# juanmc2005/diart

Hardware: NVIDIA H100
Metric: audio-seconds/sec (real-time factor) at 5s/0.5s step, batch 256 (higher is better)
Workload: dtype f32

## Files before the change

diart_b200/_lib.py:

```python
from __future__ import annotations

import ctypes as C
import os
from typing import Dict, Optional

import numpy as np
import torch

_HERE = os.path.dirname(os.path.abspath(__file__))
LIB_PATH = os.path.join(_HERE, "libdiartb200.so")

_lib: Optional[C.CDLL] = None


class DgTensor(C.Structure):
    _fields_ = [("name", C.c_char_p), ("data", C.c_void_p), ("numel", C.c_int64)]


_P = C.c_void_p
SIGNATURES = {
    "dg_last_error": (C.c_char_p, []),
    "dg_version": (C.c_int, []),
    "dg_launch_count": (C.c_int64, []),
    "dg_profile_enable": (C.c_int, [C.c_int]),
    "dg_profile_report": (C.c_int, [C.c_char_p, C.c_int]),
    "dg_selftest_gemm_tc": (C.c_int, [C.c_int, C.c_int, C.c_int, C.c_int, C.c_int, C.c_int, C.POINTER(C.c_float),
                                      C.POINTER(C.c_float)]),
    "dg_selftest_gemm_tc_grid": (C.c_int, [C.c_int, C.c_int, C.c_int, C.c_int, C.c_int, C.c_int, C.POINTER(C.c_int)]),
    "dg_selftest_gemm_tc_bounds": (C.c_int, [C.c_int, C.c_int, C.c_int, C.c_int, C.POINTER(C.c_int), C.POINTER(C.c_int),
                                             C.POINTER(C.c_int)]),
    "dg_selftest_wgmma_row_shift": (C.c_int, [C.c_int, C.POINTER(C.c_uint)]),
    "dg_selftest_gemm_tc_halo": (C.c_int, [C.c_int, C.c_int, C.c_int, C.c_int, C.c_int, C.c_int, C.POINTER(C.c_int),
                                           C.POINTER(C.c_int)]),
    "dg_selftest_split_f16_host": (C.c_int, [_P, C.c_longlong, _P, _P]),
    "dg_seg_create": (C.c_int, [C.POINTER(DgTensor), C.c_int, C.c_int, C.POINTER(_P)]),
    "dg_seg_dims": (C.c_int, [_P, C.c_int, C.POINTER(C.c_int), C.POINTER(C.c_int)]),
    "dg_seg_set_powerset": (C.c_int, [_P, C.c_int, C.c_int]),
    "dg_seg_forward": (C.c_int, [_P, _P, C.c_int, C.c_int, _P, _P]),
    "dg_seg_destroy": (C.c_int, [_P]),
    "dg_emb_create": (C.c_int, [C.POINTER(DgTensor), C.c_int, C.c_int, C.c_int, C.POINTER(_P)]),
    "dg_emb_dims": (C.c_int, [_P, C.c_int, C.POINTER(C.c_int), C.POINTER(C.c_int)]),
    "dg_emb_forward": (C.c_int, [_P, _P, _P, C.c_int, C.c_int, C.c_int, C.c_int, C.c_int, C.c_float, _P, _P]),
    "dg_emb_forward_rows": (C.c_int, [_P, _P, _P, C.c_int, C.c_int, C.c_int, _P, _P]),
    "dg_emb_destroy": (C.c_int, [_P]),
    "dg_emb_debug_trunk": (C.c_int, [_P, _P, C.c_int, C.c_int, C.c_int, _P, C.c_int64, _P]),
    "dg_seg_debug_stage": (C.c_int, [_P, _P, C.c_int, C.c_int, C.c_int, C.c_int, _P, C.c_int64, _P]),
    "dg_emb_debug_stage": (C.c_int, [_P, _P, _P, C.c_int, C.c_int, C.c_int, C.c_int, C.c_int, C.c_int, _P, C.c_int64, _P]),
    "dg_selftest_sinc_filters_host": (C.c_int, [_P, _P, _P]),
    "dg_selftest_fbank_tables_host": (C.c_int, [_P, _P]),
    "dg_osp": (C.c_int, [_P, C.c_int, C.c_int, C.c_int, C.c_float, C.c_float, C.c_int, _P, _P]),
    "dg_normalize_embeddings": (C.c_int, [_P, C.c_int, C.c_int, C.c_float, _P, _P]),
    "dg_cluster_create": (C.c_int, [C.c_int, C.c_int, C.c_double, C.c_double, C.c_double, C.c_int, C.POINTER(_P)]),
    "dg_cluster_set_metric": (C.c_int, [_P, C.c_int]),
    "dg_cluster_step": (C.c_int, [_P, _P, _P, C.c_int, C.c_int, C.c_int, _P, _P, _P]),
    "dg_cluster_reset": (C.c_int, [_P]),
    "dg_cluster_get_state": (C.c_int, [_P, _P, _P, C.POINTER(C.c_int)]),
    "dg_cluster_set_state": (C.c_int, [_P, _P, _P, C.c_int]),
    "dg_cluster_destroy": (C.c_int, [_P]),
    "dg_cluster_record_len": (C.c_int, [_P]),
    "dg_cluster_export_delta": (C.c_int, [_P, _P, _P]),
    "dg_cluster_merge": (C.c_int, [_P, _P, C.c_int, C.c_int, _P, C.c_int, _P]),
    "dg_pipeline_identity_export": (C.c_int, [_P, _P, _P]),
    "dg_pipeline_identity_merge": (C.c_int, [_P, _P, C.c_int, C.c_int, _P]),
    "dg_pipeline_create": (C.c_int, [_P, _P, _P, C.c_float, C.c_float, C.c_int, C.POINTER(_P)]),
    "dg_pipeline_set_hop": (C.c_int, [_P, C.c_int]),
    "dg_pipeline_step": (C.c_int, [_P, _P, C.c_int, C.c_int, _P, _P, _P, _P, _P]),
    "dg_pipeline_step_host": (C.c_int, [_P, _P, C.c_int, C.c_int, _P, _P, _P, _P]),
    "dg_pipeline_submit": (C.c_int, [_P, _P, C.c_int, C.c_int, _P]),
    "dg_pipeline_collect": (C.c_int, [_P, C.POINTER(_P), C.POINTER(_P), C.POINTER(_P), _P]),
    "dg_pipeline_collect_copy": (C.c_int, [_P, _P, _P, _P, _P]),
    "dg_pipeline_submit_host": (C.c_int, [_P, _P, C.c_int, C.c_int]),
    "dg_pipeline_collect_host": (C.c_int, [_P, _P, _P, _P]),
    "dg_pipeline_destroy": (C.c_int, [_P]),
    "dg_pipeline_nets_sets": (C.c_int, [_P, _P, C.c_int, C.c_int, C.c_int, _P, _P, _P, _P, C.c_int64, _P]),
    "dg_post_create": (C.c_int, [C.c_int, C.c_int, C.c_int, C.c_int, _P, C.c_double, C.c_int, C.POINTER(_P)]),
    "dg_post_step": (C.c_int, [_P, _P, _P, C.c_int, _P, _P, _P, C.c_int, C.POINTER(C.c_int), _P]),
    "dg_post_reset": (C.c_int, [_P]),
    "dg_post_destroy": (C.c_int, [_P]),
    "dg_stream_create": (C.c_int, [C.c_int, C.c_int, C.c_int, C.c_int, C.POINTER(_P)]),
    "dg_stream_push_host": (C.c_int, [_P, _P, C.c_int]),
    "dg_stream_available": (C.c_int, [_P]),
    "dg_stream_windows": (C.c_int, [_P, C.c_int, _P, _P]),
    "dg_stream_reset": (C.c_int, [_P]),
    "dg_stream_destroy": (C.c_int, [_P]),
    "dg_pipeline_submit_stream": (C.c_int, [_P, _P, C.c_int]),
    "dg_pipeline_call_stream": (C.c_int, [_P, _P, _P, C.c_int, _P, _P, _P, C.c_int, C.POINTER(C.c_int), _P, _P]),
    "dg_pipeline_call_host": (C.c_int, [_P, _P, _P, C.c_int, C.c_int, _P, _P, _P, C.c_int, C.POINTER(C.c_int), _P, _P]),
    "dg_pipeline_last_call_h2d_bytes": (C.c_int64, [_P]),
    "dg_resample_create": (C.c_int, [C.c_int, C.c_int, _P, C.c_int, C.c_int, C.POINTER(_P)]),
    "dg_resample_out_len": (C.c_int64, [_P, C.c_int64]),
    "dg_resample_forward": (C.c_int, [_P, _P, C.c_int, C.c_int64, _P, _P]),
    "dg_resample_destroy": (C.c_int, [_P]),
    "dg_stream_create_resampled": (C.c_int, [C.c_int, C.c_int, _P, C.c_int, C.c_int, C.POINTER(_P)]),
    "dg_stream_crop_host": (C.c_int, [_P, C.c_int, _P, _P]),
    "dg_sweep_create": (C.c_int, [C.c_int, C.c_int, C.c_int, C.c_int, C.c_int, _P, C.c_int, C.POINTER(_P)]),
    "dg_sweep_run": (C.c_int, [_P, _P, _P, C.c_int, _P, C.c_int, _P, _P, _P, _P, _P, C.c_int, C.POINTER(C.c_int), _P]),
    "dg_sweep_destroy": (C.c_int, [_P]),
    "dg_sweep_set_scored_regions": (C.c_int, [_P, C.c_int, _P, _P]),
    "dg_sweep_set_trial_sets": (C.c_int, [_P, C.c_int, _P, C.c_int]),
    "dg_sweep_set_seeds": (C.c_int, [_P, C.c_int, _P, _P]),
    "dg_sweep_set_identities": (C.c_int, [_P, C.c_int, _P]),
    "dg_sweep_score": (C.c_int, [_P, _P, _P, C.c_int, _P, C.c_int, _P, _P, _P, C.c_double, C.c_double, _P, _P, C.c_int,
                                 C.c_int, _P, _P, _P, C.c_int, _P]),
    "dg_sweep_run_files": (C.c_int, [_P, _P, _P, C.c_int, C.c_int, _P, _P, C.c_int, _P, _P, _P, _P, _P, C.c_int,
                                     C.POINTER(C.c_int), _P]),
    "dg_sweep_score_files": (C.c_int, [_P, _P, _P, C.c_int, C.c_int, _P, _P, C.c_int, _P, _P, _P, _P, C.c_double, _P, _P,
                                       _P, _P, _P, _P, _P, C.c_int, _P]),
    "dg_sweep_state_order": (C.c_int, [C.c_int, _P, C.c_int, _P]),
    "dg_sweep_run_latencies": (C.c_int, [_P, _P, _P, C.c_int, C.c_int, _P, C.c_int, C.c_int, _P, _P, _P, C.c_int, _P, _P,
                                         _P, _P, C.c_int, C.POINTER(C.c_int), _P]),
    "dg_sweep_score_latencies": (C.c_int, [_P, _P, _P, C.c_int, C.c_int, _P, C.c_int, C.c_int, _P, _P, _P, C.c_int, _P, _P,
                                           _P, _P, C.c_double, _P, _P, _P, _P, _P, _P]),
    "dg_sweep_check_latencies": (C.c_int, [C.c_int, C.c_int, _P, C.c_int, C.c_int, _P, _P, _P, C.c_int, C.c_int]),
    "dg_vad_sweep_curve_latencies": (C.c_int, [_P, _P, C.c_int, C.c_int, _P, C.c_int, C.c_int, _P, _P, _P, _P]),
    "dg_vad_sweep_create": (C.c_int, [C.c_int, C.c_int, C.c_int, _P, C.c_int, C.POINTER(_P)]),
    "dg_vad_sweep_curve": (C.c_int, [_P, _P, C.c_int, C.c_int, _P, _P, _P]),
    "dg_vad_sweep_run_files": (C.c_int, [_P, _P, C.c_int, _P, _P, C.c_int, C.POINTER(C.c_int), _P]),
    "dg_vad_sweep_score_files": (C.c_int, [_P, _P, C.c_int, _P, _P, _P, C.c_double, _P, _P, _P, _P]),
    "dg_vad_sweep_destroy": (C.c_int, [_P]),
    "dg_vad_sweep_set_scored_regions": (C.c_int, [_P, C.c_int, _P, _P]),
    "dg_multi_create": (C.c_int, [_P, _P, C.c_int, C.c_int, C.c_int, C.c_int, C.c_int, C.c_double, C.c_double, C.c_double,
                                  C.c_float, C.c_float, C.c_int, C.c_int, _P, C.POINTER(_P)]),
    "dg_multi_create_vad": (C.c_int, [_P, C.c_int, C.c_int, C.c_int, C.c_int, C.c_double, C.c_int, _P, C.POINTER(_P)]),
    "dg_multi_open": (C.c_int, [_P, C.c_int]),
    "dg_multi_close": (C.c_int, [_P, C.c_int]),
    "dg_multi_push_host": (C.c_int, [_P, C.c_int, _P, C.c_int]),
    "dg_multi_available": (C.c_int, [_P, C.c_int]),
    "dg_multi_step": (C.c_int, [_P, _P, C.c_int, _P, _P, _P, C.c_int, C.POINTER(C.c_int), _P, _P, _P]),
    "dg_multi_last_step_ms": (C.c_int, [_P, C.POINTER(C.c_float)]),
    "dg_multi_destroy": (C.c_int, [_P]),
    "dg_selftest_multi_staging_host": (C.c_int, [C.c_int, C.c_int, C.c_int, _P, _P, _P, _P]),
    "dg_multi_add_rate": (C.c_int, [_P, _P, C.c_int, C.c_int, C.POINTER(C.c_int)]),
    "dg_multi_open_rate": (C.c_int, [_P, C.c_int, C.c_int]),
    "dg_multi_open_config": (C.c_int, [_P, C.c_int, C.c_int, C.c_int, _P]),
    "dg_multi_open_seeded": (C.c_int, [_P, C.c_int, C.c_int, C.c_int, _P, _P, C.c_int]),
    "dg_multi_get_state": (C.c_int, [_P, C.c_int, _P, _P, C.POINTER(C.c_int)]),
    "dg_multi_last_windows": (C.c_int, [_P, _P, C.c_int]),
    "dg_gallery_create": (C.c_int, [_P, C.c_int, C.c_int, C.c_int, C.POINTER(_P)]),
    "dg_gallery_destroy": (C.c_int, [_P]),
    "dg_gallery_query": (C.c_int, [_P, _P, C.c_int, _P, _P, C.c_double, _P, _P, _P]),
    "dg_multi_set_gallery": (C.c_int, [_P, _P, C.c_double]),
    "dg_multi_set_names": (C.c_int, [_P, C.c_int, C.c_uint32, _P]),
    "dg_multi_set_slot_gallery": (C.c_int, [_P, C.c_int, _P, C.c_double]),
    "dg_selftest_gallery_plan_host": (C.c_int, [C.c_int, _P, C.c_int, _P, _P, _P, _P, _P, C.c_int, _P]),
    "dg_selftest_multi_gallery_host": (C.c_int, [C.c_int, C.c_int, C.c_int, C.c_int, _P, C.c_int, _P, _P, C.c_char_p,
                                                 C.c_int]),
    "dg_multi_last_names": (C.c_int, [_P, _P, C.c_int, C.POINTER(C.c_int)]),
    "dg_selftest_multi_frames_host": (C.c_int, [C.c_int, C.c_int, C.c_int, C.c_int, C.c_int, _P, C.c_int, _P, _P, _P, C.c_int,
                                                C.POINTER(C.c_int)]),
    "dg_multi_export_bytes": (C.c_int, [_P, _P, C.c_int, _P]),
    "dg_multi_export": (C.c_int, [_P, _P, C.c_int, C.c_int, _P, C.c_int64]),
    "dg_multi_import": (C.c_int, [_P, _P, C.c_int64, C.c_int, _P, _P]),
    "dg_selftest_multi_transfer_host": (C.c_int, [_P, C.c_int, _P, _P, _P, C.c_int, C.c_int, _P, _P, _P, C.c_int64, _P,
                                                  C.c_char_p, C.c_int]),
}


class DiartB200Error(RuntimeError):
    pass


def lib() -> C.CDLL:
    global _lib
    if _lib is not None:
        return _lib
    from . import build as _build

    if not os.path.exists(LIB_PATH) or (_build._stale() and _build.have_nvcc()):
        _build.build()
    try:
        handle = C.CDLL(LIB_PATH)
    except OSError as e:
        raise DiartB200Error(f"cannot load {LIB_PATH}: {e}. Run `python -m diart_b200.build`.") from e
    for name, (res, args) in SIGNATURES.items():
        fn = getattr(handle, name)
        fn.restype, fn.argtypes = res, args
    _lib = handle
    return handle


def check(rc: int):
    if rc == 0:
        return
    msg = lib().dg_last_error().decode()
    if rc == -1:
        if "Cannot update unknown centers" in msg:
            raise AssertionError(msg)
        raise ValueError(msg)
    if rc == -3:
        raise KeyError(msg)
    raise DiartB200Error(f"libdiartb200 error {rc}: {msg}")


def require_cuda(device: torch.device):
    if device.type != "cuda":
        raise DiartB200Error(
            f"diart_b200 runs on CUDA devices only (got '{device}'); there is no CPU implementation")
    if not torch.cuda.is_available():
        raise DiartB200Error("diart_b200 needs a CUDA device (sm_90a); none is available")


def pack_state_dict(state: Dict[str, "torch.Tensor | np.ndarray"]):
    keep, items = [], []
    for name, value in state.items():
        arr = value.detach().cpu().numpy() if isinstance(value, torch.Tensor) else np.asarray(value)
        if arr.dtype.kind != "f":
            continue
        arr = np.ascontiguousarray(arr, dtype=np.float32)
        bname = name.encode()
        keep.extend([arr, bname])
        items.append(DgTensor(bname, arr.ctypes.data, arr.size))
    array = (DgTensor * len(items))(*items)
    keep.append(array)
    return array, len(items), keep


def stream_ptr(device: torch.device) -> int:
    return torch.cuda.current_stream(device).cuda_stream


def ptr(t: Optional[torch.Tensor]) -> Optional[int]:
    return None if t is None else t.data_ptr()
```

diart_b200/csrc/api.cu:

```cuda
#include <math.h>
#include <stdlib.h>
#include <string.h>

#include <map>
#include <sstream>
#include <vector>

#include "host.cuh"

namespace dg {

static thread_local std::string g_err;
std::atomic<long long> g_launches{0};
thread_local int g_sm_limit = 0;
void set_error(const std::string& msg) { g_err = msg; }

struct ProfRec {
  std::string name;
  cudaEvent_t a, b;
};
static bool g_prof = false;
static std::vector<ProfRec> g_recs;
static const bool g_trace = getenv("DG_TRACE_LAUNCHES") && getenv("DG_TRACE_LAUNCHES")[0] == '1';
ProfScope::ProfScope(const char* name_, cudaStream_t st_) : on(g_prof), st(st_), a(nullptr), b(nullptr), name(name_) {
  if (g_trace) first = g_launches.load();
  if (!on) return;
  cudaEventCreate(&a);
  cudaEventCreate(&b);
  cudaEventRecord(a, st);
}
ProfScope::~ProfScope() {
  if (g_trace) fprintf(stderr, "dg-trace %s %lld %lld\n", name, first, (long long)g_launches.load());
  if (!on) return;
  cudaEventRecord(b, st);
  g_recs.push_back({name, a, b});
}

int upload_u16(DevBuf& b, const std::vector<uint16_t>& h) {
  if (b.ensure(h.size() * 2)) return -2;
  DG_CUDA(cudaMemcpy(b.p, h.data(), h.size() * 2, cudaMemcpyHostToDevice));
  return 0;
}

int upload_split(WeightPlanes& w, const std::vector<float>& w_nk, int N, int Npad, int K) {
  std::vector<uint16_t> h((size_t)Npad * K), l((size_t)Npad * K);
  w.scale = weight_plane_scale(w_nk.data(), (size_t)N * K);
  w.Npad = Npad;
  w.K = K;
  split_weights_host(w_nk.data(), N, Npad, K, h.data(), l.data(), w.scale);
  return (upload_u16(w.hi, h) || upload_u16(w.lo, l)) ? DG_ECUDA : 0;
}

int set_weights(TcGemm& t, const WeightPlanes& w) {
  if (t.KW * t.Cin != w.K) {
    set_error(std::string(t.tag ? t.tag : "gemm_tc") + ": the launch reads K = " + std::to_string(t.KW * t.Cin) +
              " but the weight planes have K = " + std::to_string(w.K));
    return DG_EINVAL;
  }
  t.W_hi = w.hi.p;
  t.W_lo = w.lo.p;
  t.w_scale = w.scale;
  t.Npad = w.Npad;
  return 0;
}

int upload(DevBuf& b, const std::vector<float>& h) {
  if (b.ensure(h.size() * sizeof(float))) return -2;
  DG_CUDA(cudaMemcpy(b.p, h.data(), h.size() * sizeof(float), cudaMemcpyHostToDevice));
  return 0;
}

}

extern "C" const char* dg_last_error(void) { return g_err.c_str(); }
extern "C" int dg_version(void) { return 100; }
extern "C" int64_t dg_launch_count(void) { return (int64_t)g_launches.load(); }

extern "C" int dg_profile_enable(int enable) {
  g_prof = enable != 0;
  return DG_OK;
}

extern "C" int dg_profile_report(char* buf, int cap) {
  cudaDeviceSynchronize();
  std::map<std::string, std::pair<int, double>> agg;
  for (auto& r : g_recs) {
    float ms = 0.f;
    cudaEventElapsedTime(&ms, r.a, r.b);
    auto& e = agg[r.name];
    e.first++;
    e.second += ms;
    cudaEventDestroy(r.a);
    cudaEventDestroy(r.b);
  }
  g_recs.clear();
  std::ostringstream os;
  os << "{";
  bool first = true;
  for (auto& kv : agg) {
    if (!first) os << ", ";
    first = false;
    os << "\"" << kv.first << "\": {\"count\": " << kv.second.first << ", \"ms\": " << kv.second.second << "}";
  }
  os << "}";
  const std::string s = os.str();
  if (!buf || cap <= (int)s.size()) {
    set_error("dg_profile_report: buffer too small");
    return DG_EINVAL;
  }
  memcpy(buf, s.c_str(), s.size() + 1);
  return (int)s.size();
}

extern "C" int dg_selftest_split_f16_host(const float* x, long long n, unsigned short* hi, unsigned short* lo) {
  if (!x || !hi || !lo || n < 0) {
    set_error("dg_selftest_split_f16_host: null argument");
    return DG_EINVAL;
  }
  for (long long i = 0; i < n; i++) {
    hi[i] = host_f32_to_h16(x[i]);
    lo[i] = host_f32_to_h16(x[i] - host_h16_to_f32(hi[i]));
  }
  return DG_OK;
}

extern "C" int dg_selftest_gemm_tc(int M, int Cin, int KW, int dil, int N, int epi, float* max_abs_diff,
                                   float* out_rms) {
  if (M < 1 || Cin < 16 || Cin % 16 || KW < 1 || N % 4 || !max_abs_diff || !out_rms) {
    set_error("dg_selftest_gemm_tc: bad arguments");
    return DG_EINVAL;
  }
  const int K = KW * Cin, npad = N == 64 ? 64 : (N + 255) / 256 * 256;
  const long long Mtot = M;
  std::vector<float> A((size_t)Mtot * Cin), Wkn((size_t)K * N), Wnk((size_t)N * K), bias(N), bsc(N), bsh(N);
  uint32_t seed = 12345u;
  auto rnd = [&]() {
    seed = seed * 1664525u + 1013904223u;
    return ((seed >> 8) & 0xFFFF) / 65536.f - 0.5f;
  };
  static const float amp = getenv("DG_SELFTEST_AMP") ? (float)atof(getenv("DG_SELFTEST_AMP")) : 2.f;
  for (auto& v : A) v = amp * rnd();
  for (int k = 0; k < K; k++)
    for (int n = 0; n < N; n++) {
      const float w = rnd() * 0.25f;
      Wkn[(size_t)k * N + n] = w;
      Wnk[(size_t)n * K + k] = w;
    }
  for (int n = 0; n < N; n++) {
    bias[n] = rnd();
    bsc[n] = 1.f + rnd();
    bsh[n] = rnd();
  }
  DevBuf dA, dWkn, dB, dS, dH, dAh, dAl, dC0, dC1, dOh, dOl;
  WeightPlanes dW;
  if (upload(dA, A) || upload(dWkn, Wkn) || upload(dB, bias) || upload(dS, bsc) || upload(dH, bsh) ||
      upload_split(dW, Wnk, N, npad, K))
    return DG_ECUDA;
  if (dAh.ensure((size_t)Mtot * Cin * 2) || dAl.ensure((size_t)Mtot * Cin * 2) || dC0.ensure((size_t)M * N * 4) ||
      dC1.ensure((size_t)M * N * 4) || dOh.ensure((size_t)M * N * 2) || dOl.ensure((size_t)M * N * 2))
    return DG_ECUDA;
  int rc;
  GemmArgs g{};
  g.A = dA.as<float>(); g.lda = Cin; g.Cin = Cin; g.KW = KW; g.dil = dil; g.Mtot = Mtot; g.M = M;
  g.W = dWkn.as<float>(); g.ldw = N; g.N = N; g.bias = dB.as<float>(); g.bn_scale = dS.as<float>();
  g.bn_shift = dH.as<float>(); g.C = dC0.as<float>(); g.ldc = N; g.epi = epi == 0 ? EPI_BIAS : EPI_BIAS_LEAKY_BN;
  g.tag = "selftest_simt";
  if ((rc = launch_gemm(g, nullptr))) return rc;
  if ((rc = launch_split_ex(dA.as<float>(), Mtot, Cin, Cin, Cin, 0, 1, nullptr, nullptr, dAh.p, dAl.p, nullptr))) return rc;
  TcGemm t{};
  t.A_hi = dAh.p; t.A_lo = dAl.p; t.lda = Cin; t.Cin = Cin; t.KW = KW; t.dil = dil; t.Mtot = Mtot; t.M = M;
  t.N = N; t.bias = dB.as<float>(); t.bn_scale = dS.as<float>();
  t.bn_shift = dH.as<float>(); t.out_f32 = dC1.as<float>(); t.out_hi = dOh.p; t.out_lo = dOl.p; t.ldc = N;
  t.epi = epi; t.tag = "selftest_tc";
  if ((rc = set_weights(t, dW)) || (rc = launch_gemm_tc(t, nullptr))) return rc;
  DG_CUDA(cudaDeviceSynchronize());
  std::vector<float> c0((size_t)M * N), c1((size_t)M * N);
  DG_CUDA(cudaMemcpy(c0.data(), dC0.p, c0.size() * 4, cudaMemcpyDeviceToHost));
  std::vector<uint16_t> oh, ol;
  if (epi == 1) {
    oh.resize((size_t)M * N);
    ol.resize((size_t)M * N);
    DG_CUDA(cudaMemcpy(oh.data(), dOh.p, oh.size() * 2, cudaMemcpyDeviceToHost));
    DG_CUDA(cudaMemcpy(ol.data(), dOl.p, ol.size() * 2, cudaMemcpyDeviceToHost));
    for (size_t i = 0; i < c1.size(); i++) c1[i] = host_h16_to_f32(oh[i]) + host_h16_to_f32(ol[i]);
  } else {
    DG_CUDA(cudaMemcpy(c1.data(), dC1.p, c1.size() * 4, cudaMemcpyDeviceToHost));
  }
  double md = 0, ss = 0;
  size_t worst = 0, n_big = 0;
  for (size_t i = 0; i < c0.size(); i++) {
    const double d = fabs((double)c0[i] - (double)c1[i]);
    if (!(d <= md)) {
      md = d;
      worst = i;
    }
    if (!(d <= 1e-2)) n_big++;
    ss += (double)c0[i] * c0[i];
  }
  if (n_big)
    fprintf(stderr, "dg_selftest_gemm_tc: %zu of %zu outputs differ by more than 1e-2; worst at row %zu col %zu: simt %g, wgmma %g\n",
            n_big, c0.size(), worst / N, worst % N, c0[worst], c1[worst]);
  if (n_big && epi == 1) {
    size_t shown = 0;
    for (size_t i = 0; i < c0.size() && shown < 12; i++)
      if (!(fabs((double)c0[i] - (double)c1[i]) <= 1e-2)) {
        fprintf(stderr, "   row %zu col %zu: simt %g, planes hi 0x%04x lo 0x%04x\n", i / N, i % N, c0[i], oh[i], ol[i]);
        shown++;
      }
  }
  *max_abs_diff = (float)md;
  *out_rms = (float)sqrt(ss / c0.size());
  return DG_OK;
}

extern "C" int dg_selftest_gemm_tc_grid(int M, int Cin, int KW, int dil, int N, int epi, int* equal) {
  if (M < 1 || Cin % 64 || KW < 1 || KW > 9 || N < 1 || N % 4 || epi < 0 || epi > 5 || !equal ||
      (epi == 3 && (KW != 9 || dil < 3 || M % (dil * dil) || N % 32)) || (epi == 5 && (N > 64 || M % 888))) {
    set_error("dg_selftest_gemm_tc_grid: bad arguments");
    return DG_EINVAL;
  }
  const int K = KW * Cin;
  const int npad = epi == 5 || N == 64 ? 64 : (epi == 3 && N == 32 ? 32 : (N + 127) / 128 * 128);
  const int ldc = epi == 3 ? (N + 31) / 32 * 32 : N;
  const int item_rows = epi == 4 ? 296 : 888, tile_rows = epi == 5 ? gemm_tc_pool3_tile_rows(item_rows) : 128;
  const long long m_tiles = (M + tile_rows - 1) / tile_rows;
  uint32_t seed = 777u;
  auto rnd = [&]() {
    seed = seed * 1664525u + 1013904223u;
    return ((seed >> 8) & 0xFFFF) / 65536.f - 0.5f;
  };
  std::vector<float> A((size_t)M * Cin), Wnk((size_t)N * K), bias(N), bsc(N), bsh(N), res((size_t)M * ldc), pw((size_t)M * 4);
  for (auto& v : A) v = 2.f * rnd();
  for (auto& v : Wnk) v = 0.25f * rnd();
  for (int n = 0; n < N; n++) {
    bias[n] = rnd();
    bsc[n] = 1.f + rnd();
    bsh[n] = rnd();
  }
  for (auto& v : res) v = rnd();
  for (auto& v : pw) v = rnd() + 0.5f;
  const size_t f32_bytes = epi == 0 || epi == 2 ? (size_t)M * ldc * 4 : (epi == 5 ? (size_t)(M / 3) * ldc * 4 : 0);
  const size_t plane_bytes = epi == 1 || epi == 3 ? (size_t)M * ldc * 2 : 0;
  const size_t part_bytes = epi == 4 ? (size_t)m_tiles * 2 * TC_POOL_SLOTS * N * 4 : (epi == 5 ? (size_t)m_tiles * 2 * TC_POOL3_SLOTS * N * 4 : 0);
  DevBuf dA, dAh, dAl, dB, dS, dH, dRes, dRh, dRl, dPw, dF, dOh, dOl, dPart;
  WeightPlanes dW;
  if (upload(dA, A) || upload(dB, bias) || upload(dS, bsc) || upload(dH, bsh) || upload(dRes, res) || upload(dPw, pw) ||
      upload_split(dW, Wnk, N, npad, K))
    return DG_ECUDA;
  if (dAh.ensure((size_t)M * Cin * 2) || dAl.ensure((size_t)M * Cin * 2) || dRh.ensure((size_t)M * ldc * 2) ||
      dRl.ensure((size_t)M * ldc * 2) || dF.ensure(f32_bytes + 4) || dOh.ensure(plane_bytes + 4) ||
      dOl.ensure(plane_bytes + 4) || dPart.ensure(part_bytes + 4))
    return DG_ECUDA;
  int rc;
  if ((rc = launch_split_ex(dA.as<float>(), M, Cin, Cin, Cin, 0, 1, nullptr, nullptr, dAh.p, dAl.p, nullptr)) ||
      (rc = launch_split_ex(dRes.as<float>(), M, ldc, ldc, ldc, 0, 1, nullptr, nullptr, dRh.p, dRl.p, nullptr)))
    return rc;
  int taps[9];
  for (int j = 0; j < 9; j++) taps[j] = (j / 3 - 1) * dil + (j % 3 - 1);
  TcGemm t{};
  t.A_hi = dAh.p; t.A_lo = dAl.p; t.lda = Cin; t.Cin = Cin; t.KW = KW; t.dil = dil; t.Mtot = M; t.M = M;
  t.N = N; t.bias = dB.as<float>(); t.bn_scale = dS.as<float>(); t.bn_shift = dH.as<float>(); t.ldc = ldc;
  t.epi = epi; t.tag = "selftest_tc_grid";
  t.out_f32 = f32_bytes ? dF.as<float>() : nullptr;
  t.out_hi = plane_bytes ? dOh.p : nullptr;
  t.out_lo = plane_bytes ? dOl.p : nullptr;
  if (epi == 3) {
    t.tap_off = taps; t.Wp = t.Wop = t.Hp = t.Hop = dil; t.relu = 1;
    t.res_hi = dRh.p; t.res_lo = dRl.p;
  }
  if (epi == 4) {
    t.pool_w = dPw.as<float>(); t.pool_part = dPart.as<float>(); t.pool_item_rows = item_rows; t.pool_K = 3; t.pool_T = item_rows;
  }
  if (epi == 5) {
    t.pool_part = dPart.as<float>(); t.pool_item_rows = item_rows; t.pool3_T = item_rows / 3 - 2;
    t.pool3_tile_rows = tile_rows;
  }
  if ((rc = set_weights(t, dW))) return rc;
  std::vector<unsigned char> first, cur;
  *equal = 1;
  const int caps[4] = {0, 1, 3, 7};
  for (int ci = 0; ci < 4; ci++) {
    DG_CUDA(cudaMemset(dF.p, 0, f32_bytes + 4));
    DG_CUDA(cudaMemset(dOh.p, 0, plane_bytes + 4));
    DG_CUDA(cudaMemset(dOl.p, 0, plane_bytes + 4));
    DG_CUDA(cudaMemset(dPart.p, 0, part_bytes + 4));
    {
      SmLimit cap(caps[ci]);
      if ((rc = launch_gemm_tc(t, nullptr))) return rc;
    }
    DG_CUDA(cudaDeviceSynchronize());
    cur.resize(f32_bytes + 2 * plane_bytes + part_bytes);
    DG_CUDA(cudaMemcpy(cur.data(), dF.p, f32_bytes, cudaMemcpyDeviceToHost));
    DG_CUDA(cudaMemcpy(cur.data() + f32_bytes, dOh.p, plane_bytes, cudaMemcpyDeviceToHost));
    DG_CUDA(cudaMemcpy(cur.data() + f32_bytes + plane_bytes, dOl.p, plane_bytes, cudaMemcpyDeviceToHost));
    DG_CUDA(cudaMemcpy(cur.data() + f32_bytes + 2 * plane_bytes, dPart.p, part_bytes, cudaMemcpyDeviceToHost));
    if (ci == 0)
      first.swap(cur);
    else if (cur != first)
      *equal = 0;
  }
  return DG_OK;
}

extern "C" int dg_selftest_wgmma_row_shift(int base_offset_mode, unsigned* ok_shifts) {
  if (base_offset_mode < 0 || base_offset_mode > 1 || !ok_shifts) {
    set_error("dg_selftest_wgmma_row_shift: bad arguments");
    return DG_EINVAL;
  }
  return selftest_wgmma_row_shift(base_offset_mode, ok_shifts) ? DG_ECUDA : DG_OK;
}

extern "C" int dg_selftest_gemm_tc_halo(int M, int Cin, int KW, int dil, int N, int epi, int* equal, int* halo) {
  const bool folded = Cin % 64 != 0;
  if (M < 1 || Cin < 16 || Cin % 16 || Cin > 128 || KW < 2 || KW > 9 || dil < 1 || N < 1 || N % 4 ||
      (epi != 0 && epi != 1 && epi != 2 && epi != 5) || (epi == 1 && N % 32) || (epi == 5 && (N > 64 || M % 888)) ||
      (folded && dil != 1) || !equal || !halo) {
    set_error("dg_selftest_gemm_tc_halo: bad arguments");
    return DG_EINVAL;
  }
  const int K = KW * Cin, Kf = folded ? (K + 63) / 64 * 64 : K;
  const int npad = epi == 5 || N == 64 ? 64 : (N + 127) / 128 * 128;
  const int item_rows = 888, tile_rows = epi == 5 ? gemm_tc_pool3_tile_rows(item_rows) : 128;
  const long long m_tiles = (M + tile_rows - 1) / tile_rows;
  const long long tail = 64;
  uint32_t seed = 9090u;
  auto rnd = [&]() {
    seed = seed * 1664525u + 1013904223u;
    return ((seed >> 8) & 0xFFFF) / 65536.f - 0.5f;
  };
  std::vector<float> A((size_t)(M + tail) * Cin, 0.f), Wnk((size_t)N * K), Wf((size_t)N * Kf, 0.f), bias(N), bsc(N), bsh(N);
  for (size_t i = 0; i < (size_t)M * Cin; i++) A[i] = 2.f * rnd();
  for (auto& v : Wnk) v = 0.25f * rnd();
  for (int n = 0; n < N; n++)
    for (int k = 0; k < K; k++) Wf[(size_t)n * Kf + k] = Wnk[(size_t)n * K + k];
  for (int n = 0; n < N; n++) {
    bias[n] = rnd();
    bsc[n] = 1.f + rnd();
    bsh[n] = rnd();
  }
  const size_t f32_bytes = epi == 0 || epi == 2 ? (size_t)M * N * 4 : (epi == 5 ? (size_t)(M / 3) * N * 4 : 0);
  const size_t plane_bytes = epi == 1 ? (size_t)M * N * 2 : 0;
  const size_t part_bytes = epi == 5 ? (size_t)m_tiles * 2 * TC_POOL3_SLOTS * N * 4 : 0;
  DevBuf dA, dAh, dAl, dB, dS, dH, dF, dOh, dOl, dPart;
  WeightPlanes dW, dWf;
  if (upload(dA, A) || upload(dB, bias) || upload(dS, bsc) || upload(dH, bsh) || upload_split(dW, Wnk, N, npad, K) ||
      upload_split(dWf, Wf, N, npad, Kf))
    return DG_ECUDA;
  if (dAh.ensure((size_t)(M + tail) * Cin * 2) || dAl.ensure((size_t)(M + tail) * Cin * 2) || dF.ensure(f32_bytes + 4) ||
      dOh.ensure(plane_bytes + 4) || dOl.ensure(plane_bytes + 4) || dPart.ensure(part_bytes + 4))
    return DG_ECUDA;
  int rc;
  if ((rc = launch_split_ex(dA.as<float>(), M + tail, Cin, Cin, Cin, 0, 1, nullptr, nullptr, dAh.p, dAl.p, nullptr))) return rc;
  TcGemm t{};
  t.A_hi = dAh.p; t.A_lo = dAl.p; t.lda = Cin; t.Cin = Cin; t.KW = KW; t.dil = dil; t.Mtot = M; t.M = M;
  t.N = N; t.bias = dB.as<float>(); t.bn_scale = dS.as<float>(); t.bn_shift = dH.as<float>(); t.ldc = N;
  t.epi = epi; t.tag = "selftest_tc_halo";
  t.out_f32 = f32_bytes ? dF.as<float>() : nullptr;
  t.out_hi = plane_bytes ? dOh.p : nullptr;
  t.out_lo = plane_bytes ? dOl.p : nullptr;
  if (epi == 5) {
    t.pool_part = dPart.as<float>(); t.pool_item_rows = item_rows; t.pool3_T = item_rows / 3 - 2;
    t.pool3_tile_rows = tile_rows;
  }
  if ((rc = set_weights(t, dW))) return rc;
  *halo = gemm_tc_halo(t) ? 1 : 0;
  TcGemm ref = t;
  ref.tap_boxes = 1;
  if (folded) {
    ref.Cin = Kf;
    ref.KW = 1;
    if ((rc = set_weights(ref, dWf))) return rc;
  }
  std::vector<unsigned char> first, cur;
  *equal = 1;
  for (int run = 0; run < 3; run++) {
    DG_CUDA(cudaMemset(dF.p, 0, f32_bytes + 4));
    DG_CUDA(cudaMemset(dOh.p, 0, plane_bytes + 4));
    DG_CUDA(cudaMemset(dOl.p, 0, plane_bytes + 4));
    DG_CUDA(cudaMemset(dPart.p, 0, part_bytes + 4));
    {
      SmLimit cap(run == 1 ? 3 : 0);
      if ((rc = launch_gemm_tc(run == 2 ? ref : t, nullptr))) return rc;
    }
    DG_CUDA(cudaDeviceSynchronize());
    cur.resize(f32_bytes + 2 * plane_bytes + part_bytes);
    DG_CUDA(cudaMemcpy(cur.data(), dF.p, f32_bytes, cudaMemcpyDeviceToHost));
    DG_CUDA(cudaMemcpy(cur.data() + f32_bytes, dOh.p, plane_bytes, cudaMemcpyDeviceToHost));
    DG_CUDA(cudaMemcpy(cur.data() + f32_bytes + plane_bytes, dOl.p, plane_bytes, cudaMemcpyDeviceToHost));
    DG_CUDA(cudaMemcpy(cur.data() + f32_bytes + 2 * plane_bytes, dPart.p, part_bytes, cudaMemcpyDeviceToHost));
    if (run == 0)
      first.swap(cur);
    else if (cur != first)
      *equal = 0;
  }
  return DG_OK;
}

extern "C" int dg_selftest_gemm_tc_bounds(int M, int Cin, int N, int epi, int* outside_unchanged, int* equal, int* refused) {
  const bool planes = epi == 1;
  if (M < 1 || Cin < 64 || Cin % 64 || N < 1 || N % (planes ? 32 : 4) || epi < 0 || epi > 2 || !outside_unchanged || !equal ||
      !refused) {
    set_error("dg_selftest_gemm_tc_bounds: bad arguments");
    return DG_EINVAL;
  }
  const int npad = N <= 64 && epi == 0 ? 64 : (N + 127) / 128 * 128, esize = planes ? 2 : 4;
  const int ldc = N + 40;
  const long long rows = (long long)M + 130;
  uint32_t seed = 4242u;
  auto rnd = [&]() {
    seed = seed * 1664525u + 1013904223u;
    return ((seed >> 8) & 0xFFFF) / 65536.f - 0.5f;
  };
  std::vector<float> A((size_t)M * Cin), Wnk((size_t)N * Cin), bias(N), bsc(N), bsh(N);
  for (auto& v : A) v = 2.f * rnd();
  for (auto& v : Wnk) v = 0.25f * rnd();
  for (int n = 0; n < N; n++) {
    bias[n] = rnd();
    bsc[n] = 1.f + rnd();
    bsh[n] = rnd();
  }
  const size_t dense_bytes = (size_t)M * N * esize, wide_bytes = (size_t)rows * ldc * esize + 16;
  DevBuf dA, dAh, dAl, dB, dS, dH, dD0, dD1, dW0, dW1;
  WeightPlanes dW;
  if (upload(dA, A) || upload(dB, bias) || upload(dS, bsc) || upload(dH, bsh) || upload_split(dW, Wnk, N, npad, Cin) ||
      dAh.ensure((size_t)M * Cin * 2) || dAl.ensure((size_t)M * Cin * 2) || dD0.ensure(dense_bytes) ||
      dD1.ensure(dense_bytes) || dW0.ensure(wide_bytes) || dW1.ensure(wide_bytes))
    return DG_ECUDA;
  int rc;
  if ((rc = launch_split_ex(dA.as<float>(), M, Cin, Cin, Cin, 0, 1, nullptr, nullptr, dAh.p, dAl.p, nullptr))) return rc;
  TcGemm t{};
  t.A_hi = dAh.p; t.A_lo = dAl.p; t.lda = Cin; t.Cin = Cin; t.KW = 1; t.dil = 1; t.Mtot = M; t.M = M;
  t.N = N; t.bias = dB.as<float>(); t.bn_scale = dS.as<float>(); t.bn_shift = dH.as<float>();
  t.epi = epi; t.tag = "selftest_tc_bounds";
  if ((rc = set_weights(t, dW))) return rc;
  auto point = [&](DevBuf& o0, DevBuf& o1, size_t off, int ld) {
    unsigned char* b0 = static_cast<unsigned char*>(o0.p) + off;
    unsigned char* b1 = static_cast<unsigned char*>(o1.p) + off;
    t.out_f32 = planes ? nullptr : reinterpret_cast<float*>(b0);
    t.out_hi = planes ? b0 : nullptr;
    t.out_lo = planes ? b1 : nullptr;
    t.ldc = ld;
  };
  const unsigned char SENTINEL = 0xA5;
  DG_CUDA(cudaMemset(dW0.p, SENTINEL, wide_bytes));
  DG_CUDA(cudaMemset(dW1.p, SENTINEL, wide_bytes));
  point(dD0, dD1, 0, N);
  if ((rc = launch_gemm_tc(t, nullptr))) return rc;
  point(dW0, dW1, 0, ldc);
  if ((rc = launch_gemm_tc(t, nullptr))) return rc;
  point(dW0, dW1, (size_t)esize, ldc);
  const int rc_base = launch_gemm_tc(t, nullptr);
  point(dW0, dW1, 0, ldc + (planes ? 4 : 2));
  const int rc_pitch = launch_gemm_tc(t, nullptr);
  DG_CUDA(cudaDeviceSynchronize());
  const int n_out = planes ? 2 : 1;
  std::vector<unsigned char> dense(dense_bytes), wide(wide_bytes);
  *outside_unchanged = 1;
  *equal = 1;
  for (int o = 0; o < n_out; o++) {
    DG_CUDA(cudaMemcpy(dense.data(), (o ? dD1 : dD0).p, dense_bytes, cudaMemcpyDeviceToHost));
    DG_CUDA(cudaMemcpy(wide.data(), (o ? dW1 : dW0).p, wide_bytes, cudaMemcpyDeviceToHost));
    const size_t row_bytes = (size_t)N * esize, pitch = (size_t)ldc * esize;
    for (long long r = 0; r < rows; r++) {
      const unsigned char* w = wide.data() + r * pitch;
      const bool inside = r < M;
      if (inside && memcmp(w, dense.data() + r * row_bytes, row_bytes)) *equal = 0;
      for (size_t b = inside ? row_bytes : 0; b < pitch; b++)
        if (w[b] != SENTINEL) *outside_unchanged = 0;
    }
    for (size_t b = (size_t)rows * pitch; b < wide_bytes; b++)
      if (wide[b] != SENTINEL) *outside_unchanged = 0;
  }
  *refused = rc_base == DG_EINVAL && rc_pitch == DG_EINVAL;
  return DG_OK;
}
```

diart_b200/csrc/dg_common.cuh:

```cuda
#pragma once
#include <cuda_runtime.h>
#include <stdint.h>
#include <stdio.h>

#include <atomic>
#include <string>
#include <vector>

namespace dg {

void set_error(const std::string& msg);
extern std::atomic<long long> g_launches;
extern thread_local int g_sm_limit;
inline int usable_sms() {
  int dev = 0, sms = 132;
  cudaGetDevice(&dev);
  cudaDeviceGetAttribute(&sms, cudaDevAttrMultiProcessorCount, dev);
  return (g_sm_limit > 0 && g_sm_limit < sms) ? g_sm_limit : sms;
}

#define DG_CUDA(expr)                                                                   \
  do {                                                                                  \
    cudaError_t _e = (expr);                                                            \
    if (_e != cudaSuccess) {                                                            \
      dg::set_error(std::string(#expr) + ": " + cudaGetErrorString(_e));                \
      return -2;                                                                        \
    }                                                                                   \
  } while (0)

inline bool first_use_on_device(bool* flags) {
  int dev = 0;
  cudaGetDevice(&dev);
  if (dev < 0 || dev >= 64) return true;
  if (flags[dev]) return false;
  flags[dev] = true;
  return true;
}

#define DG_LAUNCHED()                                                                   \
  do {                                                                                  \
    dg::g_launches.fetch_add(1, std::memory_order_relaxed);                             \
    cudaError_t _e = cudaGetLastError();                                                \
    if (_e != cudaSuccess) {                                                            \
      dg::set_error(std::string("kernel launch failed at ") + __FILE__ + ":" +          \
                    std::to_string(__LINE__) + ": " + cudaGetErrorString(_e));          \
      return -2;                                                                        \
    }                                                                                   \
  } while (0)

struct ProfScope {
  bool on;
  cudaStream_t st;
  cudaEvent_t a, b;
  const char* name;
  long long first = 0;
  ProfScope(const char* name, cudaStream_t st);
  ~ProfScope();
};

struct Geom {
  int S;
  int T0c;
  int T0;
  int T1;
  int T2;
  int S0, S1, S2;
};
inline Geom make_geom(int S) {
  Geom g;
  g.S = S;
  g.T0c = (S - 251) / 10 + 1;
  g.T0 = g.T0c / 3;
  g.T1 = (g.T0 - 4) / 3;
  g.T2 = (g.T1 - 4) / 3;
  g.S2 = g.T2 + 3;
  while ((g.S2 * 9) < g.T0 + 0 || (g.S2 * 3) < g.T1) g.S2++;
  g.S1 = g.S2 * 3;
  g.S0 = g.S1 * 3;
  return g;
}

__device__ __forceinline__ float leaky(float x) { return x > 0.f ? x : 0.01f * x; }

int launch_wave_stats(const float* wav, int B, int S, float* mean, float* rstd, cudaStream_t st, const int* skip_flag = nullptr);
bool stream_stats_ok(int S, int hop);
size_t stream_stats_doubles(int B, int S, int hop);
int launch_stream_stats(const float* wav, int B, int S, int hop, double* part, float* mean, float* rstd, const int* flag,
                        cudaStream_t st);
int launch_instnorm_stats(const float* x, int B, int stride_rows, int T, int C, int ldc, const float* gamma,
                          const float* beta, float* sc, float* sh, cudaStream_t st, int pool = 0, const int* skip_flag = nullptr);
int launch_instnorm_finalize(const float* part, int B, int item_rows, int tile_rows, int T, int C, int N, const float* bias,
                             const float* gamma, const float* beta, float* sc, float* sh, int ld, cudaStream_t st);
enum Epi { EPI_BIAS = 0, EPI_BIAS_LEAKY_BN = 2 };
struct GemmArgs {
  const float* A;
  int lda;
  int Cin;
  int KW, dil;
  long long Mtot;
  long long M;
  const float* W;
  int ldw;
  int N;
  const float* bias;
  const float* bn_scale;
  const float* bn_shift;
  float* C;
  int ldc;
  int epi;
  const char* tag;
};
int launch_gemm(const GemmArgs& a, cudaStream_t st);
constexpr int TC_POOL_SLOTS = 9, TC_POOL3_SLOTS = 3;
struct TcGemm {
  const void* A_hi;
  const void* A_lo;
  int lda, Cin, KW, dil;
  long long Mtot, M;
  const void* W_hi;
  const void* W_lo;
  float w_scale;
  int Npad, N;
  const float* bias;
  const float* bn_scale;
  const float* bn_shift;
  float* out_f32;
  void* out_hi;
  void* out_lo;
  int ldc;
  int epi;
  const char* tag;
  const int* tap_off;
  int Wp, Hp, Wop, Hop, stride2, relu;
  const void* res_hi;
  const void* res_lo;
  const float* pool_w;
  float* pool_part;
  int pool_item_rows, pool_K;
  int pool_T;
  int pool3_T, pool3_tile_rows;
  int tap_boxes;
};
inline int gemm_tc_pool3_tile_rows(int item_rows) {
  for (int t = 126; t >= 96; t -= 3)
    if (item_rows % t == 0) return t;
  return 0;
}
int launch_gemm_tc(const TcGemm& g, cudaStream_t st);
bool gemm_tc_halo(const TcGemm& g);
int selftest_wgmma_row_shift(int base_offset_mode, unsigned* ok_shifts);
int launch_split_ex(const float* x, long long rows_out, int C, int ld_in, int ld_out, int pool, int item_rows,
                    const float* sc, const float* sh, void* hi, void* lo, cudaStream_t st, const int* skip_flag = nullptr);
void split_weights_host(const float* w, int N, int Npad, int K, uint16_t* hi, uint16_t* lo, float scale = 1.f);
float weight_plane_scale(const float* w, size_t n);
uint16_t host_f32_to_h16(float f);
float host_h16_to_f32(uint16_t h);
int sinc_tc_rows_per_item(const Geom& g);
size_t sinc_tc_plane_elems(int B, const Geom& g);
void sinc_tc_pack_filters(const float* filt, uint16_t* planes );
void sinc_tc_affine_consts(const float* filt, float beta, float* cf);
int launch_sinc_prep(const float* wav, const float* mean, const float* rstd, int B, const Geom& g, void* planes_hi,
                     void* planes_lo, cudaStream_t st, const int* skip_flag = nullptr);
int launch_sinc0_tc(float gamma, const float* cf_dev, const void* w_planes, int B, const Geom& g, const void* planes_hi,
                    const void* planes_lo, float* p0, cudaStream_t st, const int* skip_flag = nullptr);
struct SincStreamGeom {
  int Ls;
  int P;
  int rows;
  size_t plane;
};
SincStreamGeom sinc_stream_geom(int B, const Geom& g, int hop);
int launch_overlap_check(const float* wav, int B, int S, int hop, int* flag, cudaStream_t st);
int launch_stream_prep(const float* wav, const float* rstd, int B, const Geom& g, int hop, void* planes_hi, void* planes_lo,
                       int* flag, cudaStream_t st);
int launch_sinc0_tc_stream(const void* w_planes, int B, const Geom& g, int hop, const void* planes_hi, const void* planes_lo,
                           float* craw, const int* flag, cudaStream_t st);
size_t sinc_pool_part_floats(int B, const Geom& g, int hop);
int launch_sinc_pool_fused(const float* craw, const float* mean, const float* rstd, const float* cf, const float* hsum, float gamma,
                           int B, const Geom& g, int hop, const float* g0, const float* b0, float* part, float* sc, float* sh,
                           void* planes_hi, void* planes_lo, const int* flag, cudaStream_t st);
size_t lstm_tc_plane_elems();
int lstm_tc_rows(int B);
int lstm_tc_ctas(int B);
float lstm_tc_pack_whh(const float* whh_fwd, const float* whh_bwd, uint16_t* hi, uint16_t* lo);
int launch_lstm_layer_tc(const float* gx, const void* whh_hi, const void* whh_lo, float w_scale, int B, int T, int stride,
                         float* hout, void* out_hi, void* out_lo, cudaStream_t st);
int launch_seg_final(const float* y , const float* wc , const float* bc, int B, int T,
                     int stride, int K, float* seg , cudaStream_t st);
int launch_seg_powerset(const float* y, const float* wc, const float* bc, int B, int T, int stride, int C, int num_speakers,
                        const unsigned* masks_dev, float* seg , cudaStream_t st);
int launch_osp(const float* seg, int B, int F, int K, float gamma, float beta, int normalize, float* out,
               cudaStream_t st);
constexpr int DG_MAX_OSP_SETS = 64;
struct OspSets {
  float gamma[DG_MAX_OSP_SETS], beta[DG_MAX_OSP_SETS];
  int normalize[DG_MAX_OSP_SETS];
};
int launch_osp_sets(const float* seg, int B, int F, int K, const OspSets& sets, int G, float* out, cudaStream_t st);
int launch_stats_pool(const float* x , int B, int stride, int T, int C, const float* w ,
                      int F, int K, const int* idx0, const int* idx1, const float* lam1, float eps,
                      float* pooled , cudaStream_t st, long long item_pitch = 0, int row_pitch = 0);
int launch_pool_weights(const float* w , int B, int F, int K, int item_rows, int T, const int* idx0, const int* idx1,
                        const float* lam1, float eps, float* row_w , float* vsum , cudaStream_t st);
int launch_pool_weights_sets(const float* w, int B, int G, int F, int K, int item_rows, int T, const int* idx0, const int* idx1,
                             const float* lam1, float eps, float* row_w, long long rw_stride, float* vsum, cudaStream_t st);
int launch_pool_finalize(const float* part, const float* row_w, const float* vsum, const float* pivot, int B, int K, int C,
                         int item_rows, int T, float eps, float* pooled , cudaStream_t st);
int launch_l2norm(const float* in, int rows, int D, float norm, float* out, cudaStream_t st);
int launch_row_equal_flags(const float* wav, int N, int S, int* flags, cudaStream_t st);
int launch_gather_rows(const float* src, const int* index, int rows, int cols, float* dst, cudaStream_t st);
int launch_fb_planes(const float* wav, int B, int S, void* hi, void* lo, float* inv_scale, float* level, cudaStream_t st);
int launch_fb_mel(const float* spec, int ld, int rows_per_item, int T, int B, const float* inv_scale, const float* level,
                  const float* banks, const int* k_lo, const int* k_hi, float* logmel, cudaStream_t st);
int launch_fb_mean(const float* logmel, int B, int T, float* mean, cudaStream_t st);
int launch_rn_stem(const float* logmel, const float* mean, int B, int T, const float* w, const float* sc, const float* sh,
                   void* hi, void* lo, cudaStream_t st);
struct ClusterParams {
  int M, D;
  float tau_f, rho_f;
  double delta;
  int metric;
};
int launch_cluster_step(const ClusterParams& p, const float* seg, const float* emb, int B, int F, int K,
                        double* centers, int* active, int* initialized, float* prep ,
                        double* prep_d , int32_t* map, float* permuted, cudaStream_t st);
int launch_cluster_export(const double* centers, const int* active, const double* base, const int* base_active, int M,
                          int D, double* record, cudaStream_t st);
int launch_cluster_merge(const double* records, int world, int rank, const ClusterParams& p, int rec_len, double* centers,
                         int* active, double* base, int* base_active, int* initialized, int32_t* relabel,
                         cudaStream_t st);
int launch_relabel_maps(int32_t* maps, int n, const int32_t* relabel, cudaStream_t st);
int launch_cluster_sweep(const ClusterParams& p, const double* trials_dev, int T, const int2* states_dev, int S,
                         const int* chunk_off_dev, const float* seg, const float* emb, int B, int F, int K, double* centers,
                         int* active, int* initialized, float* prep, double* prep_d, int32_t* maps, cudaStream_t st,
                         bool own_rows = false);
int launch_cluster_sweep_sets(const ClusterParams& p, const double* trials_dev, int T, const int2* states_dev, int S,
                              const int* chunk_off_dev, const float* seg, const float* emb, int G, int B, int F, int K,
                              double* centers, int* active, int* initialized, float* prep, double* prep_d, int32_t* maps,
                              cudaStream_t st);
size_t cluster_prep_floats(int B, int K);
int launch_sweep_seed(const int* seed_off, const double* seeds, int nf, int T, int M, int D, double* centers, int* active,
                      int* initialized, cudaStream_t st);
int launch_post_virtual(const float* seg, const int32_t* map, int N, const int32_t* vchunk, int Nv, int F, int K, int M, int nw,
                        const int32_t* plan, int plan_stride, const double* hamming, const double* taus, int T,
                        int32_t* header, uint32_t* turns, int turn_cap, unsigned int* total, cudaStream_t st);
int launch_expand_windows(const float* ring, long long r0, int C, int hop, int S, int B, float* wav, cudaStream_t st);
struct RingPiece {
  long long src, dst;
  int slot, n;
};
struct TickSlot {
  int slot, row0, n, cur, n_hist, nw, pad[2];
};
int launch_ring_scatter(const float* staged, const RingPiece* pieces, int n_pieces, int C, float* rings, cudaStream_t st);
int launch_ring_gather(const float* rings, int C, const TickSlot* act, const int2* rows, const long long* start, int S, int B,
                       float* wav, cudaStream_t st);
int launch_post_slots(const float* seg, const int32_t* map, const float* hist_seg, const int32_t* hist_map,
                      const TickSlot* act, const int2* rows, int slots, int B, int F, int K, int M, int nw,
                      const int32_t* plan, int plan_stride, const double* hamming, const double* params, int32_t* header,
                      uint32_t* turns, int turn_cap, unsigned int* total, cudaStream_t st);
int launch_post_slots_history(const float* seg, const int32_t* map, float* hist_seg, int32_t* hist_map, const TickSlot* act,
                              int n_act, int slots, int F, int K, int nw, cudaStream_t st);
size_t cluster_prep_doubles(int B, int K);
int launch_der_hyp_count(const int32_t* header, const uint32_t* turns, int nf, const int* chunk_off, int T, int N, int M,
                         const double* out_start, const double* out_res, const double* shifts, double collar, int* offsets,
                         cudaStream_t st);
int launch_der_hyp_write(const int32_t* header, const uint32_t* turns, int nf, const int* chunk_off, int T, int N, int M,
                         const double* out_start, const double* out_res, const double* shifts, double collar, int* offsets,
                         double* segs, double* segs_copy, int copy_cap, cudaStream_t st);
constexpr int DER_ROFF = 33;
int launch_der_score(const int* hoff, const double* hseg, int nf, int T, int M, const int* roff, const int* R,
                     const double* rseg, double* comp, cudaStream_t st, const int* uoff = nullptr,
                     const double* useg = nullptr, const int* named = nullptr);
int launch_vad_curve_virtual(const float* seg, const int32_t* vchunk, int Nv, int F, int K, const int32_t* plan, int plan_stride,
                             const double* hamming, const long long* curve_off, double* curve, cudaStream_t st);
int launch_vad_binarize(const double* curve, const long long* curve_off, int N, int T, const double* taus, int32_t* header,
                        uint32_t* turns, int turn_cap, unsigned int* total, cudaStream_t st);
int launch_vad_slots(const float* seg, const float* hist_vad, const TickSlot* act, const int2* rows, int slots, int B, int F,
                     int K, int nw, const int32_t* plan, int plan_stride, const double* hamming, const double* params,
                     int32_t* header, uint32_t* turns, int turn_cap, unsigned int* total, cudaStream_t st);
int launch_vad_slots_history(const float* seg, float* hist_vad, const TickSlot* act, int n_act, int slots, int F, int K, int nw,
                             cudaStream_t st);
struct RsGeom {
  int o, n, w, T;
};
struct RsItem {
  long long start, len, j_lo, j_cnt, out_off;
};
struct RsJob {
  const float* x;
  long long C;
  const RsItem* items;
  RsItem base;
  long long start_step, out_step;
  const float* W;
  RsGeom g;
  float* out;
};
long long resample_out_len(const RsGeom& g, long long L);
bool resample_geom_ok(const RsGeom& g);
int launch_resample(const RsJob& j, int items, long long max_out, cudaStream_t st);
int launch_resample_stream(const float* ring, long long C, long long rpos, long long hop, long long L, int B, const float* W,
                           const RsGeom& g, float* ys, float* out, cudaStream_t st);
struct RsFrames {
  long long first;
  int slot, count;
};
struct RsRow {
  long long start, frame0;
  int slot, row;
};
int launch_resample_frames(const float* rings, long long C, const RsFrames* items, int n_items, long long max_count,
                           const float* W, const RsGeom& g, float* yrings, long long Y, long long Q, cudaStream_t st);
int launch_resample_gather(const float* rings, long long C, const float* yrings, long long Y, long long Q, const RsRow* rows,
                           int n_rows, long long r_lo, long long r_hi, const float* W, const RsGeom& g, long long L,
                           long long out_len, float* wav, cudaStream_t st);

void fbank_frame_operator(std::vector<float>& op );
void fbank_mel_banks(std::vector<float>& banks , std::vector<int>& k_lo, std::vector<int>& k_hi);

constexpr int GAL_TILE_E = 64, GAL_TILE_Q = 128, GAL_KC = 16, GAL_NAME_PREFIX = 1024;
struct GalGroup {
  const double* E;
  const double* En;
  double threshold;
  int G, tiles, per_split, splits, q_ub, seg0, seg1, pad;
};
struct GalWork {
  int group, tile, split;
};
int launch_gallery_norms(const double* E, int G, int Dp, double* En, cudaStream_t st);
int gallery_plan(std::vector<GalGroup>& groups, std::vector<GalWork>& work);
int launch_gallery_nearest(const GalGroup* groups, const GalWork* work, int n_work, const int2* gq, int Dp, const double* X,
                           int D, const int2* qd, int Qmax, const int32_t* claimed, double* part_d, int* part_e,
                           cudaStream_t st);
int launch_gallery_queries(const int2* segs, int n, const GalGroup* groups, int n_groups, const int* active,
                           const uint32_t* named, int M, int2* qd, int* seg_off, int2* gq, int* names, cudaStream_t st);
int launch_gallery_claim(const double* part_d, const int* part_e, int Qmax, const int2* qd, const int* seg_off,
                         const int2* segs, int n_seg, const GalGroup* groups, int32_t* claimed, int32_t* entry_out,
                         double* dist_out, uint32_t* named, int M, int* names, int32_t* list, int32_t* prefix, cudaStream_t st);

struct XferPiece {
  const uint32_t* src;
  uint32_t* dst;
  long long n, src_pos, src_mod, dst_pos, dst_mod;
};
int launch_slot_transfer(const XferPiece* pieces, int n_pieces, const char* tag, cudaStream_t st);

}
```

diart_b200/csrc/gemm_tc.cu:

```cuda
#include <cuda.h>
#include <cuda_bf16.h>
#include <math.h>
#include <stdlib.h>
#include <string.h>

#include <algorithm>
#include <map>
#include <mutex>
#include <string>
#include <utility>
#include <vector>

#include "dg_common.cuh"
#include "tc_ptx.cuh"

namespace dg {

constexpr int TC_BM = 128, TC_BK = 32, TC_THREADS = 384;
constexpr int TC_SMEM_MAX = 227 * 1024;

struct TcArgs {
  long long M;
  int N;
  int m_tiles, n_tiles;
  int KW, dil, cin_blocks;
  const float* bias;
  const float* bn_scale;
  const float* bn_shift;
  float* out_f32;
  __nv_bfloat16* out_hi;
  __nv_bfloat16* out_lo;
  int ldc;
  float acc_scale;
  int tap_off[9];
  int Wp, Hp, Wop, Hop, stride2, relu;
  const __nv_bfloat16* res_hi;
  const __nv_bfloat16* res_lo;
  const float* pool_w;
  float* pool_part;
  int pool_item_rows, pool_K, pool_T;
  int tile_rows, pool3_T;
  unsigned* tile_ctr;
  int halo_rows;
  int cin;
  int wblocks;
  int halo_bytes;
  int op_bytes;
};

enum TcEpi { TC_BIAS_F32 = 0, TC_LEAKY_BN_SPLIT = 1, TC_LEAKY_BN_F32 = 2, TC_CONV2D = 3, TC_POOL = 4, TC_MAXPOOL3 = 5 };

__host__ __device__ constexpr bool tc_pooling(int epi) { return epi == TC_POOL || epi == TC_MAXPOOL3; }
__host__ __device__ constexpr bool tc_box_store(int epi) { return epi == TC_BIAS_F32 || epi == TC_LEAKY_BN_SPLIT || epi == TC_LEAKY_BN_F32; }

template <int BN>
struct TcSmem {
  static constexpr int A_BYTES = TC_BM * TC_BK * 2;
  static constexpr int W_BYTES = BN * TC_BK * 2;
  static constexpr int STAGE_BYTES = 2 * A_BYTES + 2 * W_BYTES;
  static constexpr int W_STAGE_BYTES = 2 * W_BYTES;
  static constexpr int NSTAGE = BN == 128 ? 4 : 6;
  static constexpr int NSTAGE_HALO = BN == 128 ? 5 : 6;
  __host__ static int halo_bytes(int cin, int rows) { return (2 * ((cin + 31) / 32) * rows * 64 + 1023) / 1024 * 1024; }
  __host__ static int halo_op_bytes(int cin, int rows) { return 2 * halo_bytes(cin, rows) + NSTAGE_HALO * W_STAGE_BYTES; }
  static constexpr int BAR_BYTES = 256;
  static constexpr int PARAM_FLOATS = 3 * BN;
  static constexpr int CHUNK_W = 64;
  static constexpr int CHUNK_FLOATS = CHUNK_W / 32 * TC_BM * 33;
  __host__ __device__ static constexpr int extra_floats(int epi) { return epi == TC_POOL ? 128 * 4 + 4 * 2 * 8 * 32 : (epi == TC_MAXPOOL3 ? 4 * 2 * 2 * 32 : 0); }
  __host__ __device__ static constexpr int consumer_floats(int epi) { return PARAM_FLOATS + (tc_pooling(epi) ? CHUNK_FLOATS + extra_floats(epi) : 0); }
  static constexpr int ACC_LD = BN + 4;
  static constexpr int BOX_BYTES = TC_BM * 128;
  __host__ __device__ static constexpr int stage_tile_bytes(int epi) {
    return tc_pooling(epi) ? 0 : (epi == TC_CONV2D ? TC_BM * ACC_LD * 4 : TC_BM * BN * 4);
  }
  __host__ __device__ static constexpr int total(int epi, int op_bytes = NSTAGE * STAGE_BYTES) {
    return op_bytes + stage_tile_bytes(epi) + BAR_BYTES + 2 * consumer_floats(epi) * 4 + 1024;
  }
};
static_assert(TcSmem<128>::total(TC_POOL) <= TC_SMEM_MAX && TcSmem<64>::total(TC_MAXPOOL3) <= TC_SMEM_MAX &&
              TcSmem<128>::total(TC_CONV2D) <= TC_SMEM_MAX && TcSmem<64>::total(TC_CONV2D) <= TC_SMEM_MAX &&
              TcSmem<32>::total(TC_CONV2D) <= TC_SMEM_MAX && TcSmem<128>::total(TC_BIAS_F32) <= TC_SMEM_MAX,
              "gemm_tc: shared memory");

template <int BN, int EPI>
__device__ __forceinline__ void tc_stage_params(const TcArgs& a, float* params, int bar, int n0, int et) {
  named_sync(bar, 128);
  for (int i = et; i < BN; i += 128) {
    const int n = n0 + i;
    const bool ok = n < a.N;
    params[i] = (ok && a.bias) ? a.bias[n] : 0.f;
    constexpr bool has_bn = EPI != TC_BIAS_F32;
    params[BN + i] = (ok && has_bn) ? a.bn_scale[n] * (EPI == TC_CONV2D ? a.acc_scale : 1.f) : 1.f;
    params[2 * BN + i] = (ok && has_bn) ? a.bn_shift[n] : 0.f;
  }
  named_sync(bar, 128);
}

template <int BN, int EPI>
__device__ __forceinline__ void tc_box_epilogue(const TcArgs& a, const float* params, float (&acc)[2][BN / 2],
                                                uint32_t tile, int quad, int lane) {
  using S = TcSmem<BN>;
  const int r0 = 16 * quad + (lane >> 2), sw = lane >> 2, cq = lane & 3;
#pragma unroll
  for (int j = 0; j < BN / 8; j++) {
    const int col = 8 * j + 2 * cq;
    const float2 bias = *reinterpret_cast<const float2*>(params + col);
    float2 bsc = make_float2(1.f, 1.f), bsh = make_float2(0.f, 0.f);
    if (EPI != TC_BIAS_F32) {
      bsc = *reinterpret_cast<const float2*>(params + BN + col);
      bsh = *reinterpret_cast<const float2*>(params + 2 * BN + col);
    }
#pragma unroll
    for (int h = 0; h < 2; h++) {
#pragma unroll
      for (int e2 = 0; e2 < 2; e2++) {
        const int row = 64 * h + r0 + 8 * e2;
        float x0 = fmaf(acc[h][4 * j + 2 * e2], a.acc_scale, bias.x);
        float x1 = fmaf(acc[h][4 * j + 2 * e2 + 1], a.acc_scale, bias.y);
        if (EPI != TC_BIAS_F32) {
          x0 = fmaf(leaky(x0), bsc.x, bsh.x);
          x1 = fmaf(leaky(x1), bsc.y, bsh.y);
        }
        if (EPI == TC_LEAKY_BN_SPLIT) {
          uint16_t h0, l0, h1, l1;
          split_h16(x0, h0, l0);
          split_h16(x1, h1, l1);
          const int off = (j / 8) * S::BOX_BYTES + row * 128 + (((j & 7) ^ sw) << 4) + 4 * cq;
          st_shared_u32(tile + off, pack_u16x2(h0, h1));
          st_shared_u32(tile + (BN / 64) * S::BOX_BYTES + off, pack_u16x2(l0, l1));
        } else {
          const int q = 2 * (j & 3) + (cq >> 1);
          const int off = (j / 4) * S::BOX_BYTES + row * 128 + ((q ^ sw) << 4) + 8 * (cq & 1);
          st_shared_v2(tile + off, x0, x1);
        }
      }
    }
  }
}

__device__ __forceinline__ void acc_ld32(const float* p, uint32_t (&r)[32]) {
#pragma unroll
  for (int i = 0; i < 8; i++) {
    const float4 v = reinterpret_cast<const float4*>(p)[i];
    r[4 * i] = __float_as_uint(v.x);
    r[4 * i + 1] = __float_as_uint(v.y);
    r[4 * i + 2] = __float_as_uint(v.z);
    r[4 * i + 3] = __float_as_uint(v.w);
  }
}

template <int BN>
__device__ __forceinline__ void tc_conv2d_epilogue_tile(const TcArgs& a, const float* params, const float* acc_row,
                                                        long long mt, int n0, int quad, int lane) {
    const long long m = mt * TC_BM + quad * 32 + lane;
    long long mo = m;
    bool row_ok = m < a.M;
    {
      const unsigned mu = (unsigned)m, per = (unsigned)(a.Wp * a.Hp);
      const unsigned item = mu / per, rem = mu - item * per;
      const int w = (int)(rem / (unsigned)a.Hp), h = (int)(rem - (unsigned)w * (unsigned)a.Hp);
      row_ok = row_ok && w >= 1 && w <= a.Wp - 2 && h >= 1 && h <= a.Hp - 2;
      if (a.stride2) {
        row_ok = row_ok && (w & 1) && (h & 1);
        mo = ((long long)item * a.Wop + ((w - 1) >> 1) + 1) * a.Hop + ((h - 1) >> 1) + 1;
      }
    }
#pragma unroll 1
    for (int c = 0; c < BN; c += 32) {
      uint32_t r[32];
      acc_ld32(acc_row + c, r);
      if (n0 + c >= a.N) continue;
      float v[32];
#pragma unroll
      for (int i = 0; i < 32; i++) v[i] = fmaf(__uint_as_float(r[i]), params[BN + c + i], params[2 * BN + c + i]);
      if (row_ok && a.res_hi) {
        const uint4* rh = reinterpret_cast<const uint4*>(a.res_hi + mo * a.ldc + n0 + c);
        const uint4* rl = reinterpret_cast<const uint4*>(a.res_lo + mo * a.ldc + n0 + c);
#pragma unroll
        for (int q = 0; q < 4; q++) {
          const uint4 hq = rh[q], lq = rl[q];
          const uint32_t hw[4] = {hq.x, hq.y, hq.z, hq.w}, lw[4] = {lq.x, lq.y, lq.z, lq.w};
#pragma unroll
          for (int e = 0; e < 4; e++) {
            v[8 * q + 2 * e] += h16_to_f32((uint16_t)(hw[e] & 0xFFFFu)) + h16_to_f32((uint16_t)(lw[e] & 0xFFFFu));
            v[8 * q + 2 * e + 1] += h16_to_f32((uint16_t)(hw[e] >> 16)) + h16_to_f32((uint16_t)(lw[e] >> 16));
          }
        }
      }
      if (a.relu) {
#pragma unroll
        for (int i = 0; i < 32; i++) v[i] = fmaxf(v[i], 0.f);
      }
      if (row_ok) {
        if (a.out_f32) {
          float* po = a.out_f32 + mo * a.ldc + n0 + c;
#pragma unroll
          for (int i = 0; i < 8; i++)
            reinterpret_cast<float4*>(po)[i] = make_float4(v[4 * i], v[4 * i + 1], v[4 * i + 2], v[4 * i + 3]);
        }
        if (a.out_hi) {
          uint32_t hi[16], lo[16];
#pragma unroll
          for (int i = 0; i < 16; i++) {
            uint16_t h0, l0, h1, l1;
            split_h16(v[2 * i], h0, l0);
            split_h16(v[2 * i + 1], h1, l1);
            hi[i] = pack_u16x2(h0, h1);
            lo[i] = pack_u16x2(l0, l1);
          }
          uint4* ph = reinterpret_cast<uint4*>(a.out_hi + mo * a.ldc + n0 + c);
          uint4* pl = reinterpret_cast<uint4*>(a.out_lo + mo * a.ldc + n0 + c);
#pragma unroll
          for (int i = 0; i < 4; i++) {
            ph[i] = make_uint4(hi[4 * i], hi[4 * i + 1], hi[4 * i + 2], hi[4 * i + 3]);
            pl[i] = make_uint4(lo[4 * i], lo[4 * i + 1], lo[4 * i + 2], lo[4 * i + 3]);
          }
        }
      }
    }
}

template <int BN, int EPI>
__device__ __forceinline__ void tc_pool_epilogue_tile(const TcArgs& a, float* params, float* chunk, float* pool_stage,
                                                 const float (&acc)[2][BN / 2], int bar, long long mt, int n0, int quad,
                                                 int lane, int et, bool stage_params) {
    const long long m = mt * (EPI == TC_MAXPOOL3 ? a.tile_rows : TC_BM) + quad * 32 + lane;
    if (stage_params) {
      named_sync(bar, 128);
      for (int i = et; i < BN; i += 128) {
        const int n = n0 + i;
        const bool ok = n < a.N;
        params[i] = (ok && a.bias) ? a.bias[n] : 0.f;
        constexpr bool has_bn = EPI != TC_BIAS_F32 && EPI != TC_MAXPOOL3;
        params[BN + i] = (ok && has_bn) ? a.bn_scale[n] : 1.f;
        params[2 * BN + i] = (ok && has_bn) ? a.bn_shift[n] : 0.f;
      }
      named_sync(bar, 128);
    }
    int brow = TC_BM, valid0 = 0, valid1 = 0;
    if (EPI == TC_POOL) {
      float4 pw = make_float4(0.f, 0.f, 0.f, 0.f);
      if (m < a.M) pw = *reinterpret_cast<const float4*>(a.pool_w + m * 4);
      reinterpret_cast<float4*>(pool_stage)[quad * 32 + lane] = pw;
      const long long first = (long long)mt * TC_BM;
      const long long nxt = (first / a.pool_item_rows + 1) * a.pool_item_rows;
      brow = nxt - first < TC_BM ? (int)(nxt - first) : TC_BM;
      valid0 = min(brow, max(0, a.pool_T - (a.pool_item_rows - (int)(nxt - first))));
      valid1 = max(0, min(TC_BM - brow, a.pool_T));
      named_sync(bar, 128);
    }
    constexpr int CW = TcSmem<BN>::CHUNK_W;
    const int fr0 = 16 * quad + (lane >> 2), fc0 = 2 * (lane & 3);
#pragma unroll
    for (int c0 = 0; c0 < BN; c0 += CW) {
      {
#pragma unroll
        for (int c = c0; c < c0 + CW; c += 32) {
          float* dsm = chunk + (c - c0) / 32 * (128 * 33);
#pragma unroll
          for (int jj = 0; jj < 4; jj++) {
#pragma unroll
            for (int e1 = 0; e1 < 2; e1++) {
              const int col = 8 * jj + fc0 + e1;
              float bb = 0.f, ss = 0.f, hh = 0.f;
              if (EPI == TC_POOL) bb = params[c + col], ss = params[BN + c + col], hh = params[2 * BN + c + col];
#pragma unroll
              for (int h = 0; h < 2; h++) {
#pragma unroll
                for (int e2 = 0; e2 < 2; e2++) {
                  const float y = acc[h][4 * (c / 8 + jj) + 2 * e2 + e1];
                  float* d = dsm + (64 * h + fr0 + 8 * e2) * 33 + col;
                  if (EPI == TC_POOL) {
                    const float x = leaky(fmaf(y, a.acc_scale, bb));
                    *d = fmaf(x, ss, hh) - hh;
                  } else {
                    *d = y * a.acc_scale;
                  }
                }
              }
            }
          }
        }
      }
      named_sync(bar, 128);
#pragma unroll
      for (int c = c0; c < c0 + CW; c += 32) {
        if (EPI == TC_POOL) {
          const float* dsm = chunk + (c - c0) / 32 * (128 * 33);
          const float4* wsm = reinterpret_cast<const float4*>(pool_stage);
          float* stg = pool_stage + 128 * 4;
          const int col = et & 31;
          auto pivot = [&](int lo, int n) {
            if (n <= 0) return 0.f;
            const float pa = dsm[lo * 33 + col], pb = dsm[(lo + n / 2) * 33 + col];
            return fabsf(pa + pb) > 16.f * fabsf(pa - pb) ? 0.5f * (pa + pb) : 0.f;
          };
          if (c != c0) named_sync(bar, 128);
          {
            const int rg = et >> 5, r_lo = rg * 32, r_hi = r_lo + 32;
#pragma unroll
            for (int sg = 0; sg < 2; sg++) {
              const int lo = sg == 0 ? r_lo : max(r_lo, brow), hi = sg == 0 ? min(r_hi, brow) : r_hi;
              const float piv = sg ? pivot(brow < TC_BM ? brow : 0, valid1) : pivot(0, valid0);
              float s1[4] = {0.f, 0.f, 0.f, 0.f}, s2[4] = {0.f, 0.f, 0.f, 0.f};
              if (a.pool_K <= 3) {
#pragma unroll 8
                for (int rr = lo; rr < hi; rr++) {
                  const float dv = dsm[rr * 33 + col] - piv;
                  const float4 w4 = wsm[rr];
                  const float a0 = w4.x * dv, a1 = w4.y * dv, a2 = w4.z * dv;
                  s1[0] += a0; s1[1] += a1; s1[2] += a2;
                  s2[0] = fmaf(a0, dv, s2[0]); s2[1] = fmaf(a1, dv, s2[1]); s2[2] = fmaf(a2, dv, s2[2]);
                }
              } else {
#pragma unroll 8
                for (int rr = lo; rr < hi; rr++) {
                  const float dv = dsm[rr * 33 + col] - piv;
                  const float4 w4 = wsm[rr];
                  const float a0 = w4.x * dv, a1 = w4.y * dv, a2 = w4.z * dv, a3 = w4.w * dv;
                  s1[0] += a0; s1[1] += a1; s1[2] += a2; s1[3] += a3;
                  s2[0] = fmaf(a0, dv, s2[0]); s2[1] = fmaf(a1, dv, s2[1]); s2[2] = fmaf(a2, dv, s2[2]); s2[3] = fmaf(a3, dv, s2[3]);
                }
              }
#pragma unroll
              for (int k = 0; k < 4; k++) {
                stg[((rg * 2 + sg) * 8 + 2 * k) * 32 + col] = s1[k];
                stg[((rg * 2 + sg) * 8 + 2 * k + 1) * 32 + col] = s2[k];
              }
            }
          }
          named_sync(bar, 128);
          {
            const int twoK = 2 * a.pool_K, n = n0 + c + col;
            for (int q = et >> 5; q < 2 * twoK; q += 4) {
              const int sg = q >= twoK ? 1 : 0, j = q - sg * twoK;
              const float tot = ((stg[((0 * 2 + sg) * 8 + j) * 32 + col] + stg[((1 * 2 + sg) * 8 + j) * 32 + col]) +
                                 stg[((2 * 2 + sg) * 8 + j) * 32 + col]) + stg[((3 * 2 + sg) * 8 + j) * 32 + col];
              if (n < a.N && mt < a.m_tiles) a.pool_part[(((size_t)mt * 2 + sg) * TC_POOL_SLOTS + j) * a.N + n] = tot;
            }
            if (et < 64 && n < a.N && mt < a.m_tiles) {
              const int sg = et >> 5;
              a.pool_part[(((size_t)mt * 2 + sg) * TC_POOL_SLOTS + 8) * a.N + n] = sg ? pivot(brow < TC_BM ? brow : 0, valid1)
                                                                                      : pivot(0, valid0);
            }
          }
          if (c + 32 == c0 + CW) named_sync(bar, 128);
          continue;
        }
        if (EPI == TC_MAXPOOL3) {
          const float* dsm = chunk + (c - c0) / 32 * (128 * 33);
          float* stg = pool_stage;
          {
            const int col = et & 31, rg = et >> 5, n = n0 + c + col;
            const long long first = mt * (long long)a.tile_rows;
            const long long item0 = first / a.pool_item_rows;
            const long long nxt = (item0 + 1) * a.pool_item_rows;
            const int brow3 = nxt - first < a.tile_rows ? (int)(nxt - first) / 3 : a.tile_rows / 3;
            const long long p_first = first / 3;
            const int f0 = (int)(p_first - item0 * (a.pool_item_rows / 3));
            const long long Mp = a.M / 3;
            const float bias = params[c + col];
            auto pooled = [&](int pr) {
              return fmaxf(fmaxf(dsm[(3 * pr) * 33 + col], dsm[(3 * pr + 1) * 33 + col]), dsm[(3 * pr + 2) * 33 + col]);
            };
            const float piv0 = pooled(0), piv1 = pooled(brow3 < a.tile_rows / 3 ? brow3 : 0);
            float s1[2] = {0.f, 0.f}, s2[2] = {0.f, 0.f};
            for (int pr = rg; pr < a.tile_rows / 3; pr += 4) {
              const float v = pooled(pr);
              const int sg = pr >= brow3 ? 1 : 0;
              const int frame = sg ? pr - brow3 : f0 + pr;
              const long long P = p_first + pr;
              if (P < Mp) {
                if (n < a.N) a.out_f32[P * a.ldc + n] = v + bias;
                if (frame < a.pool3_T) {
                  const float dv = v - (sg ? piv1 : piv0);
                  s1[sg] += dv;
                  s2[sg] = fmaf(dv, dv, s2[sg]);
                }
              }
            }
#pragma unroll
            for (int sg = 0; sg < 2; sg++) {
              stg[((rg * 2 + sg) * 2 + 0) * 32 + col] = s1[sg];
              stg[((rg * 2 + sg) * 2 + 1) * 32 + col] = s2[sg];
            }
            if (rg == 0 && n < a.N)
#pragma unroll
              for (int sg = 0; sg < 2; sg++) a.pool_part[(((size_t)mt * 2 + sg) * TC_POOL3_SLOTS + 2) * a.N + n] = sg ? piv1 : piv0;
          }
          named_sync(bar, 128);
          {
            const int col = et & 31, q = et >> 5, sg = q >> 1, j = q & 1, n = n0 + c + col;
            const float tot = ((stg[((0 * 2 + sg) * 2 + j) * 32 + col] + stg[((1 * 2 + sg) * 2 + j) * 32 + col]) +
                               stg[((2 * 2 + sg) * 2 + j) * 32 + col]) + stg[((3 * 2 + sg) * 2 + j) * 32 + col];
            if (n < a.N) a.pool_part[(((size_t)mt * 2 + sg) * TC_POOL3_SLOTS + j) * a.N + n] = tot;
          }
          named_sync(bar, 128);
          continue;
        }
      }
    }
}

template <int BN, int EPI, bool HALO>
__global__ void __launch_bounds__(TC_THREADS, 1)
gemm_tc_kernel(const __grid_constant__ CUtensorMap tmA_hi, const __grid_constant__ CUtensorMap tmA_lo,
               const __grid_constant__ CUtensorMap tmW_hi, const __grid_constant__ CUtensorMap tmW_lo,
               const __grid_constant__ CUtensorMap tmC0, const __grid_constant__ CUtensorMap tmC1, TcArgs a) {
  using S = TcSmem<BN>;
  constexpr bool POOLING = tc_pooling(EPI);
  constexpr int NSTAGE = HALO ? S::NSTAGE_HALO : S::NSTAGE;
  extern __shared__ unsigned char smem_raw[];
  unsigned char* smem = reinterpret_cast<unsigned char*>((reinterpret_cast<uintptr_t>(smem_raw) + 1023) & ~uintptr_t(1023));
  unsigned char* ring = HALO ? smem + 2 * a.halo_bytes : smem;
  constexpr int RING_STAGE = HALO ? S::W_STAGE_BYTES : S::STAGE_BYTES;
  unsigned char* tile_s = smem + a.op_bytes;
  uint64_t* bars = reinterpret_cast<uint64_t*>(tile_s + S::stage_tile_bytes(EPI));
  uint64_t* full = bars;
  uint64_t* empty = bars + NSTAGE;
  uint64_t* tile_full = bars + 2 * NSTAGE;
  uint64_t* tile_empty = tile_full + 2;
  uint64_t* halo_full = tile_empty + 2;
  uint64_t* halo_empty = halo_full + 2;
  volatile int* tile_idx = reinterpret_cast<volatile int*>(halo_empty + 2);
  float* cons = reinterpret_cast<float*>(reinterpret_cast<unsigned char*>(bars) + S::BAR_BYTES);

  const int warp = __shfl_sync(0xffffffffu, (int)(threadIdx.x >> 5), 0), lane = threadIdx.x & 31;
  const int wg = warp >> 2;
  const int num_tiles = a.m_tiles * a.n_tiles;
  const int kblocks = HALO ? a.wblocks : a.KW * a.cin_blocks;
  const int halo_box = a.halo_rows * 64, halo_cb = (a.cin + 31) / 32;

  if (threadIdx.x == 0) {
    for (int s = 0; s < NSTAGE; s++) {
      mbar_init(&full[s], 1);
      mbar_init(&empty[s], 1);
    }
    for (int c = 0; c < 2; c++) {
      mbar_init(&tile_full[c], 1);
      mbar_init(&tile_empty[c], 128);
      mbar_init(&halo_full[c], 1);
      mbar_init(&halo_empty[c], 1);
    }
    asm volatile("fence.mbarrier_init.release.cluster;" ::: "memory");
  }
  __syncthreads();

  if (wg == 0) {
    setmaxnreg_dec<HALO ? 48 : 40>();
    if (threadIdx.x == 0) {
      int stage = 0, phase = 0, next = 0;
      bool halo_next = false;
      for (int i = 0, tile = blockIdx.x;; i++) {
        const int c = i & 1;
        mbar_wait(&tile_empty[c], ((i >> 1) & 1) ^ 1);
        if (tile >= num_tiles) {
          tile_idx[c] = -1;
          mbar_arrive(&tile_full[c]);
          mbar_wait(&tile_empty[c ^ 1], (((i + 1) >> 1) & 1) ^ 1);
          tile_idx[c ^ 1] = -2;
          mbar_arrive(&tile_full[c ^ 1]);
          break;
        }
        tile_idx[c] = tile;
        mbar_arrive(&tile_full[c]);
        const int mt = tile / a.n_tiles, nt = tile - mt * a.n_tiles;
        const int m0 = mt * (EPI == TC_MAXPOOL3 ? a.tile_rows : TC_BM), n0 = nt * BN;
        if constexpr (HALO) {
          auto load_halo = [&](int cc, int r0) {
            unsigned char* hs = smem + cc * a.halo_bytes;
            mbar_expect_tx(&halo_full[cc], 2 * halo_cb * halo_box);
            for (int cb = 0; cb < halo_cb; cb++) {
              tma_load_2d(hs + cb * halo_box, &tmA_hi, cb * TC_BK, r0, &halo_full[cc]);
              tma_load_2d(hs + (halo_cb + cb) * halo_box, &tmA_lo, cb * TC_BK, r0, &halo_full[cc]);
            }
          };
          if (!halo_next) {
            mbar_wait(&halo_empty[c], ((i >> 1) & 1) ^ 1);
            load_halo(c, m0);
          }
          halo_next = false;
          next = POOLING ? (int)gridDim.x + (int)atomicAdd(&a.tile_ctr[0], 1u) : tile + (int)gridDim.x;
          const int next_m0 = next / a.n_tiles * (EPI == TC_MAXPOOL3 ? a.tile_rows : TC_BM);
          const uint32_t next_par = (((i + 1) >> 1) & 1) ^ 1;
          for (int kb = 0; kb < kblocks; kb++) {
            const long long t0 = clock64();
            for (;;) {
              if (!halo_next && next < num_tiles && mbar_test_wait(&halo_empty[c ^ 1], next_par)) {
                load_halo(c ^ 1, next_m0);
                halo_next = true;
              }
              if (mbar_test_wait(&empty[stage], phase ^ 1)) break;
              if (clock64() - t0 > 4000000000LL) __trap();
            }
            unsigned char* st = ring + stage * RING_STAGE;
            mbar_expect_tx(&full[stage], S::W_STAGE_BYTES);
            tma_load_2d(st, &tmW_hi, kb * TC_BK, n0, &full[stage]);
            tma_load_2d(st + S::W_BYTES, &tmW_lo, kb * TC_BK, n0, &full[stage]);
            if (++stage == NSTAGE) {
              stage = 0;
              phase ^= 1;
            }
          }
        }
        for (int j = 0; j < (HALO ? 0 : a.KW); j++) {
          for (int cb = 0; cb < a.cin_blocks; cb++) {
            mbar_wait(&empty[stage], phase ^ 1);
            unsigned char* st = smem + stage * S::STAGE_BYTES;
            mbar_expect_tx(&full[stage], S::STAGE_BYTES);
            const int kcol = (j * a.cin_blocks + cb) * TC_BK;
            tma_load_2d(st, &tmA_hi, cb * TC_BK, m0 + a.tap_off[j], &full[stage]);
            tma_load_2d(st + S::A_BYTES, &tmA_lo, cb * TC_BK, m0 + a.tap_off[j], &full[stage]);
            tma_load_2d(st + 2 * S::A_BYTES, &tmW_hi, kcol, n0, &full[stage]);
            tma_load_2d(st + 2 * S::A_BYTES + S::W_BYTES, &tmW_lo, kcol, n0, &full[stage]);
            if (++stage == NSTAGE) {
              stage = 0;
              phase ^= 1;
            }
          }
        }
        if (!HALO) next = POOLING ? (int)gridDim.x + (int)atomicAdd(&a.tile_ctr[0], 1u) : tile + (int)gridDim.x;
        tile = next;
      }
      if (POOLING) {
        __threadfence();
        if (atomicAdd(&a.tile_ctr[1], 1u) == gridDim.x - 1) {
          atomicExch(&a.tile_ctr[0], 0u);
          atomicExch(&a.tile_ctr[1], 0u);
        }
      }
    }
    return;
  }
  setmaxnreg_inc<HALO ? 224 : 232>();
  const int c = wg - 1, quad = warp & 3, et = threadIdx.x - 128 * wg;
  float* params = cons + c * S::consumer_floats(EPI);
  float* chunk = params + S::PARAM_FLOATS;
  float* pool_stage = chunk + S::CHUNK_FLOATS;
  const int bar = 1 + c, turn = 3 + c, turn_other = 3 + (c ^ 1), acc_free = 5 + c, acc_free_other = 5 + (c ^ 1);
  if (c == 1) {
    named_arrive(3, 256);
    if (!POOLING) named_arrive(5, 256);
  }
  for (int n = 0;; n++) {
    mbar_wait(&tile_full[c], n & 1);
    const int tile = tile_idx[c];
    mbar_arrive(&tile_empty[c]);
    if (tc_box_store(EPI) && tile >= 0 && (a.n_tiles > 1 || n == 0))
      tc_stage_params<BN, EPI>(a, params, bar, (tile - tile / a.n_tiles * a.n_tiles) * BN, et);
    named_sync(turn, 256);
    if (tile < 0) {
      if (tile == -1) {
        named_arrive(turn_other, 256);
        if (!POOLING) named_sync(acc_free, 256);
      }
      break;
    }
    const int pos = (2 * n + c) * kblocks;
    int stage = pos % NSTAGE, phase = (pos / NSTAGE) & 1;
    float acc[2][BN / 2];
#pragma unroll
    for (int i = 0; i < BN / 2; i++) acc[0][i] = acc[1][i] = 0.f;
    uint32_t htap = 0;
    int hch = 0;
    if constexpr (HALO) mbar_wait(&halo_full[c], n & 1);
    const uint32_t hs = smem_u32(smem + c * a.halo_bytes);
    for (int kb = 0; kb < kblocks; kb++) {
      mbar_wait(&full[stage], phase);
      const uint32_t sa = smem_u32(ring + stage * RING_STAGE);
      const uint32_t sw = HALO ? sa : sa + 2 * S::A_BYTES;
      const uint64_t w_hi = wg_desc_sw64(sw), w_lo = wg_desc_sw64(sw + S::W_BYTES);
      constexpr uint64_t HALF = (uint64_t)((64 * TC_BK * 2) >> 4);
      wg_fence_acc(acc[0]);
      wg_fence_acc(acc[1]);
      wg_fence();
#pragma unroll
      for (int ks = 0; ks < TC_BK / 16; ks++) {
        const uint64_t adv = (uint64_t)((ks * 32) >> 4);
        uint64_t a_hi, a_lo;
        if constexpr (HALO) {
          const uint32_t aa = hs + (uint32_t)(hch >> 5) * halo_box + (uint32_t)(hch & 31) * 2 + htap;
          a_hi = wg_desc_sw64(aa);
          a_lo = wg_desc_sw64(aa + halo_cb * halo_box);
          hch += 16;
          const bool next_tap = hch == a.cin;
          hch = next_tap ? 0 : hch;
          htap += next_tap ? a.dil * 64 : 0;
        } else {
          a_hi = wg_desc_sw64(sa) + adv;
          a_lo = wg_desc_sw64(sa + S::A_BYTES) + adv;
        }
#pragma unroll
        for (int h = 0; h < 2; h++) {
          wgmma_ss<BN>(acc[h], a_lo + h * HALF, w_hi + adv, (kb | ks) != 0);
          wgmma_ss<BN>(acc[h], a_hi + h * HALF, w_lo + adv, 1);
          wgmma_ss<BN>(acc[h], a_hi + h * HALF, w_hi + adv, 1);
        }
      }
      wg_commit();
      wg_wait<1>();
      wg_fence_acc(acc[0]);
      wg_fence_acc(acc[1]);
      if (kb > 0 && et == 0) mbar_arrive(&empty[stage == 0 ? NSTAGE - 1 : stage - 1]);
      if (++stage == NSTAGE) {
        stage = 0;
        phase ^= 1;
      }
    }
    named_arrive(turn_other, 256);
    wg_wait<0>();
    wg_fence_acc(acc[0]);
    wg_fence_acc(acc[1]);
    if (et == 0) mbar_arrive(&empty[stage == 0 ? NSTAGE - 1 : stage - 1]);
    if (HALO && et == 0) mbar_arrive(&halo_empty[c]);
    const int mt = tile / a.n_tiles, nt = tile - mt * a.n_tiles;
    const bool stage_params = a.n_tiles > 1 || n == 0;
    if constexpr (POOLING) {
      tc_pool_epilogue_tile<BN, EPI>(a, params, chunk, pool_stage, acc, bar, mt, nt * BN, quad, lane, et, stage_params);
    } else if constexpr (EPI == TC_CONV2D) {
      float* acc_s = reinterpret_cast<float*>(tile_s);
      named_sync(acc_free, 256);
#pragma unroll
      for (int h = 0; h < 2; h++) {
        const int r0 = 64 * h + 16 * quad + (lane >> 2);
#pragma unroll
        for (int j = 0; j < BN / 8; j++) {
          const int col = 8 * j + 2 * (lane & 3);
          *reinterpret_cast<float2*>(acc_s + r0 * S::ACC_LD + col) = make_float2(acc[h][4 * j], acc[h][4 * j + 1]);
          *reinterpret_cast<float2*>(acc_s + (r0 + 8) * S::ACC_LD + col) = make_float2(acc[h][4 * j + 2], acc[h][4 * j + 3]);
        }
      }
      named_sync(bar, 128);
      if (stage_params) tc_stage_params<BN, EPI>(a, params, bar, nt * BN, et);
      tc_conv2d_epilogue_tile<BN>(a, params, acc_s + et * S::ACC_LD, mt, nt * BN, quad, lane);
      named_arrive(acc_free_other, 256);
    } else {
      named_sync(acc_free, 256);
      tc_box_epilogue<BN, EPI>(a, params, acc, smem_u32(tile_s), quad, lane);
      fence_proxy_async_smem();
      named_sync(bar, 128);
      if (et == 0) {
        const int m0 = mt * TC_BM, n0 = nt * BN;
        if (EPI == TC_LEAKY_BN_SPLIT) {
#pragma unroll
          for (int b = 0; b < BN / 64; b++) {
            if (n0 + 64 * b >= a.N) break;
            tma_store_2d(&tmC0, tile_s + b * S::BOX_BYTES, n0 + 64 * b, m0);
            tma_store_2d(&tmC1, tile_s + (BN / 64 + b) * S::BOX_BYTES, n0 + 64 * b, m0);
          }
        } else {
#pragma unroll
          for (int b = 0; b < BN / 32; b++) {
            if (n0 + 32 * b >= a.N) break;
            tma_store_2d(&tmC0, tile_s + b * S::BOX_BYTES, n0 + 32 * b, m0);
          }
        }
        bulk_commit();
        bulk_wait_read_all();
      }
      __syncwarp();
      named_arrive(acc_free_other, 256);
    }
  }
  if (tc_box_store(EPI) && et == 0) bulk_wait_all();
}

static int make_map(CUtensorMap* m, const void* base, long long rows, int cols, int ld, int box_cols, int box_rows,
                    bool f32 = false) {
  EncodeTiledFn fn = encode_fn();
  if (!fn) {
    set_error("cuTensorMapEncodeTiled is not available from the driver");
    return -2;
  }
  const int esize = f32 ? 4 : 2;
  cuuint64_t dims[2] = {(cuuint64_t)cols, (cuuint64_t)rows};
  cuuint64_t strides[1] = {(cuuint64_t)ld * esize};
  cuuint32_t box[2] = {(cuuint32_t)box_cols, (cuuint32_t)box_rows};
  cuuint32_t estr[2] = {1, 1};
  CUresult r = fn(m, f32 ? CU_TENSOR_MAP_DATA_TYPE_FLOAT32 : CU_TENSOR_MAP_DATA_TYPE_BFLOAT16, 2, const_cast<void*>(base), dims,
                  strides, box, estr, CU_TENSOR_MAP_INTERLEAVE_NONE,
                  box_cols * esize == 128 ? CU_TENSOR_MAP_SWIZZLE_128B : CU_TENSOR_MAP_SWIZZLE_64B,
                  CU_TENSOR_MAP_L2_PROMOTION_L2_256B, CU_TENSOR_MAP_FLOAT_OOB_FILL_NONE);
  if (r != CUDA_SUCCESS) {
    set_error("cuTensorMapEncodeTiled failed with code " + std::to_string((int)r));
    return -2;
  }
  return 0;
}

constexpr int TC_CTR_SLOTS = 1024;
__device__ unsigned g_tc_tile_ctr[TC_CTR_SLOTS][2];

static unsigned* tile_counter(cudaStream_t st) {
  static std::mutex mu;
  static std::map<std::pair<int, cudaStream_t>, int> slot_of;
  static int used[64] = {};
  int dev = 0;
  if (cudaGetDevice(&dev) != cudaSuccess || dev < 0 || dev >= 64) {
    set_error("gemm_tc: no current CUDA device");
    return nullptr;
  }
  int slot;
  {
    std::lock_guard<std::mutex> lock(mu);
    auto it = slot_of.find({dev, st});
    if (it != slot_of.end()) {
      slot = it->second;
    } else {
      if (used[dev] == TC_CTR_SLOTS) {
        set_error("gemm_tc: more than " + std::to_string(TC_CTR_SLOTS) + " streams have launched GEMMs on one device");
        return nullptr;
      }
      slot = slot_of[{dev, st}] = used[dev]++;
    }
  }
  void* base = nullptr;
  if (cudaGetSymbolAddress(&base, g_tc_tile_ctr) != cudaSuccess) {
    set_error("gemm_tc: cannot address the tile counters");
    return nullptr;
  }
  return static_cast<unsigned*>(base) + 2 * slot;
}

static int tc_bn(const TcGemm& g) { return g.epi == TC_MAXPOOL3 || (g.Npad == 64 && g.epi == TC_BIAS_F32) ? 64 : 128; }
static int tc_halo_rows(const TcGemm& g) {
  return (TC_BM + (g.KW - ((g.KW * g.Cin) % 32 ? 0 : 1)) * g.dil + 7) / 8 * 8;
}
template <int BN>
static int tc_halo_smem(const TcGemm& g) { return TcSmem<BN>::total(g.epi, TcSmem<BN>::halo_op_bytes(g.Cin, tc_halo_rows(g))); }

bool gemm_tc_halo(const TcGemm& g) {
  if (g.tap_boxes || g.epi == TC_CONV2D || g.tap_off || g.KW < 2 || g.dil < 1 || g.Cin % 16 || g.Cin > 128 ||
      tc_halo_rows(g) > 256)
    return false;
  return (tc_bn(g) == 64 ? tc_halo_smem<64>(g) : tc_halo_smem<128>(g)) <= TC_SMEM_MAX;
}

static int tc_setup(const TcGemm& g, int bn, int epi, bool halo, CUtensorMap* maps, TcArgs& a) {
  const int Ktot = g.KW * g.Cin, bk = TC_BK, a_rows = halo ? tc_halo_rows(g) : TC_BM;
  if (make_map(&maps[0], g.A_hi, g.Mtot, g.Cin, g.lda, bk, a_rows) || make_map(&maps[1], g.A_lo, g.Mtot, g.Cin, g.lda, bk, a_rows) ||
      make_map(&maps[2], g.W_hi, g.Npad, Ktot, Ktot, bk, bn) || make_map(&maps[3], g.W_lo, g.Npad, Ktot, Ktot, bk, bn))
    return -2;
  memset(&maps[4], 0, 2 * sizeof(CUtensorMap));
  if (epi == TC_LEAKY_BN_SPLIT) {
    if (make_map(&maps[4], g.out_hi, g.M, g.N, g.ldc, 64, TC_BM) || make_map(&maps[5], g.out_lo, g.M, g.N, g.ldc, 64, TC_BM))
      return -2;
  } else if (tc_box_store(epi)) {
    if (make_map(&maps[4], g.out_f32, g.M, g.N, g.ldc, 32, TC_BM, true)) return -2;
  }
  a = TcArgs{};
  a.M = g.M; a.N = g.N; a.n_tiles = (g.N + bn - 1) / bn;
  a.tile_rows = epi == TC_MAXPOOL3 ? g.pool3_tile_rows : TC_BM;
  a.pool3_T = g.pool3_T;
  a.m_tiles = (int)((g.M + a.tile_rows - 1) / a.tile_rows);
  a.KW = g.KW; a.dil = g.dil; a.cin_blocks = g.Cin / bk;
  a.bias = g.bias; a.bn_scale = g.bn_scale; a.bn_shift = g.bn_shift;
  a.out_f32 = g.out_f32; a.out_hi = reinterpret_cast<__nv_bfloat16*>(g.out_hi);
  a.out_lo = reinterpret_cast<__nv_bfloat16*>(g.out_lo); a.ldc = g.ldc;
  a.acc_scale = g.w_scale > 0.f ? 1.f / g.w_scale : 1.f;
  for (int j = 0; j < 9; j++) a.tap_off[j] = j < g.KW ? (g.tap_off ? g.tap_off[j] : j * g.dil) : 0;
  a.Wp = g.Wp; a.Hp = g.Hp; a.Wop = g.Wop; a.Hop = g.Hop; a.stride2 = g.stride2; a.relu = g.relu;
  a.res_hi = reinterpret_cast<const __nv_bfloat16*>(g.res_hi);
  a.res_lo = reinterpret_cast<const __nv_bfloat16*>(g.res_lo);
  a.pool_w = g.pool_w; a.pool_part = g.pool_part; a.pool_item_rows = g.pool_item_rows; a.pool_K = g.pool_K; a.pool_T = g.pool_T;
  a.cin = g.Cin;
  if (halo) {
    a.halo_rows = a_rows;
    a.wblocks = (Ktot + bk - 1) / bk;
    a.halo_bytes = bn == 64 ? TcSmem<64>::halo_bytes(g.Cin, a_rows) : TcSmem<128>::halo_bytes(g.Cin, a_rows);
    a.op_bytes = bn == 64 ? TcSmem<64>::halo_op_bytes(g.Cin, a_rows) : TcSmem<128>::halo_op_bytes(g.Cin, a_rows);
  } else {
    a.op_bytes = bn == 128 ? TcSmem<128>::NSTAGE * TcSmem<128>::STAGE_BYTES
                           : (bn == 64 ? TcSmem<64>::NSTAGE * TcSmem<64>::STAGE_BYTES : TcSmem<32>::NSTAGE * TcSmem<32>::STAGE_BYTES);
  }
  return 0;
}

static int tc_grid(const TcArgs& a) {
  const int sms = usable_sms();
  const int tiles = a.m_tiles * a.n_tiles;
  return tiles < sms ? tiles : sms;
}

template <int BN, int EPI, bool HALO>
static int launch_tc(const TcGemm& g, cudaStream_t st) {
  using S = TcSmem<BN>;
  CUtensorMap m[6];
  TcArgs a;
  if (tc_setup(g, BN, EPI, HALO, m, a)) return -2;
  if (tc_pooling(EPI) && !(a.tile_ctr = tile_counter(st))) return -2;
  auto kern = gemm_tc_kernel<BN, EPI, HALO>;
  static bool attr_done[64] = {};
  if (first_use_on_device(attr_done))
    DG_CUDA(cudaFuncSetAttribute(kern, cudaFuncAttributeMaxDynamicSharedMemorySize, HALO ? TC_SMEM_MAX : S::total(EPI)));
  kern<<<tc_grid(a), TC_THREADS, S::total(EPI, a.op_bytes), st>>>(m[0], m[1], m[2], m[3], m[4], m[5], a);
  DG_LAUNCHED();
  return 0;
}

template <int BN, int EPI>
static int launch_tc(const TcGemm& g, cudaStream_t st) {
  return gemm_tc_halo(g) ? launch_tc<BN, EPI, true>(g, st) : launch_tc<BN, EPI, false>(g, st);
}

int launch_gemm_tc(const TcGemm& g, cudaStream_t st) {
  ProfScope _ps(g.tag ? g.tag : "gemm_tc", st);
  if (g.Cin % (gemm_tc_halo(g) ? 16 : 64) || g.lda % 8 || g.ldc % (g.epi == TC_LEAKY_BN_SPLIT ? 8 : 4) ||
      (g.Npad % 128 && g.Npad != 64 && g.Npad != 32) || g.KW < 1 || g.KW > 9) {
    set_error("gemm_tc: Cin must be a multiple of 64 (a Conv1d of 2..9 taps over at most 128 channels whose tile halo fits "
              "in shared memory, e.g. Cin 80: a multiple of 16), A pitch a multiple of 8, output pitch a multiple of 4 "
              "(8 for 16-bit planes), padded N 32, 64 or a multiple of 128, at most 9 taps");
    return -1;
  }
  if (g.epi == TC_LEAKY_BN_SPLIT && g.N % 32) {
    set_error("gemm_tc (planes): N must be a multiple of 32");
    return -1;
  }
  if (tc_box_store(g.epi)) {
    const bool planes = g.epi == TC_LEAKY_BN_SPLIT;
    const uintptr_t base = planes ? ((uintptr_t)g.out_hi | (uintptr_t)g.out_lo) : (uintptr_t)g.out_f32;
    if (!base || (planes && (!g.out_hi || !g.out_lo)) || base % 16 || g.ldc < g.N || g.M >= (1LL << 31)) {
      set_error("gemm_tc: the output needs a 16-byte aligned base, a pitch of at least N and fewer than 2^31 rows");
      return -1;
    }
  }
  if (g.epi == TC_CONV2D) {
    if (g.ldc % 32 || g.N % 32 || g.Wp < 3 || g.Hp < 3 || (!g.out_hi && !g.out_f32) || g.M >= (1LL << 31)) {
      set_error("gemm_tc (conv2d): channel counts must be multiples of 32");
      return -1;
    }
    if (g.Npad == 32) return launch_tc<32, TC_CONV2D, false>(g, st);
    if (g.Npad == 64) return launch_tc<64, TC_CONV2D, false>(g, st);
    return launch_tc<128, TC_CONV2D, false>(g, st);
  }
  if (g.epi == TC_POOL) {
    if (g.Npad % 128 || !g.pool_w || !g.pool_part || g.pool_K < 1 || g.pool_K > 4 || g.pool_item_rows < TC_BM || g.pool_T < 1 ||
        g.pool_T > g.pool_item_rows) {
      set_error("gemm_tc (pool): needs 128-wide tiles, 1..4 speakers, items of at least 128 rows and 1..item rows valid frames");
      return -1;
    }
    return launch_tc<128, TC_POOL>(g, st);
  }
  if (g.epi == TC_MAXPOOL3) {
    if (g.Npad != 64 || !g.out_f32 || !g.pool_part || g.pool3_T < 1 || g.pool3_tile_rows < 3 || g.pool3_tile_rows > 126 ||
        g.pool3_tile_rows % 3 || g.pool_item_rows % g.pool3_tile_rows || g.M % g.pool_item_rows) {
      set_error("gemm_tc (maxpool3): needs 64 output channels and tiles of 3..126 rows (a multiple of 3) that divide the item");
      return -1;
    }
    return launch_tc<64, TC_MAXPOOL3>(g, st);
  }
  if (g.Npad == 64 && g.epi == TC_BIAS_F32) return launch_tc<64, TC_BIAS_F32>(g, st);
  switch (g.epi) {
    case TC_BIAS_F32:
      return launch_tc<128, TC_BIAS_F32>(g, st);
    case TC_LEAKY_BN_SPLIT:
      return launch_tc<128, TC_LEAKY_BN_SPLIT>(g, st);
    default:
      return launch_tc<128, TC_LEAKY_BN_F32>(g, st);
  }
}

__global__ void __launch_bounds__(128) wgmma_row_shift_kernel(const __grid_constant__ CUtensorMap tmA,
                                                              const __grid_constant__ CUtensorMap tmW, int base_offset_mode,
                                                              float* out) {
  __shared__ __align__(1024) unsigned char sm[72 * 64 + 8 * 64];
  __shared__ uint64_t bar;
  if (threadIdx.x == 0) {
    mbar_init(&bar, 1);
    asm volatile("fence.mbarrier_init.release.cluster;" ::: "memory");
  }
  __syncthreads();
  if (threadIdx.x == 0) {
    mbar_expect_tx(&bar, sizeof(sm));
    tma_load_2d(sm, &tmA, 0, 0, &bar);
    tma_load_2d(sm + 72 * 64, &tmW, 0, 0, &bar);
  }
  mbar_wait(&bar, 0);
  const int w = threadIdx.x >> 5, l = threadIdx.x & 31;
  for (int r = 0; r <= 8; r++) {
    for (int ks = 0; ks < 2; ks++) {
      const uint32_t sa = smem_u32(sm) + r * 64 + ks * 32;
      uint64_t da = wg_desc_sw64(sa);
      if (base_offset_mode) da |= (uint64_t)((sa >> 7) & 7) << 49;
      const uint64_t dw = wg_desc_sw64(smem_u32(sm + 72 * 64) + ks * 32);
      float d[4] = {0.f, 0.f, 0.f, 0.f};
      wg_fence_acc(d);
      wg_fence();
      wgmma_ss<8>(d, da, dw, 0);
      wg_commit();
      wg_wait<0>();
      wg_fence_acc(d);
      for (int i = 0; i < 4; i++)
        out[((r * 2 + ks) * 64 + 16 * w + l / 4 + 8 * ((i / 2) % 2)) * 8 + 2 * (l % 4) + i % 2] = d[i];
    }
  }
}

int selftest_wgmma_row_shift(int base_offset_mode, unsigned* ok_shifts) {
  std::vector<uint16_t> A(72 * 32), W(8 * 32);
  std::vector<float> Af(A.size()), Wf(W.size());
  for (size_t i = 0; i < A.size(); i++) Af[i] = (float)((int)((i * 7 + i / 32 * 3) % 9) - 4);
  for (size_t i = 0; i < W.size(); i++) Wf[i] = (float)((int)((i * 5 + 1) % 7) - 3);
  for (size_t i = 0; i < A.size(); i++) A[i] = host_f32_to_h16(Af[i]);
  for (size_t i = 0; i < W.size(); i++) W[i] = host_f32_to_h16(Wf[i]);
  void *dA = nullptr, *dW = nullptr, *dO = nullptr;
  const size_t out_n = 9 * 2 * 64 * 8;
  int rc = 0;
  CUtensorMap mA, mW;
  if (cudaMalloc(&dA, A.size() * 2) != cudaSuccess || cudaMalloc(&dW, W.size() * 2) != cudaSuccess ||
      cudaMalloc(&dO, out_n * 4) != cudaSuccess ||
      cudaMemcpy(dA, A.data(), A.size() * 2, cudaMemcpyHostToDevice) != cudaSuccess ||
      cudaMemcpy(dW, W.data(), W.size() * 2, cudaMemcpyHostToDevice) != cudaSuccess) {
    set_error("selftest_wgmma_row_shift: device buffers");
    rc = -2;
  }
  if (!rc && (make_map(&mA, dA, 72, 32, 32, 32, 72) || make_map(&mW, dW, 8, 32, 32, 32, 8))) rc = -2;
  std::vector<float> out(out_n);
  if (!rc) {
    wgmma_row_shift_kernel<<<1, 128>>>(mA, mW, base_offset_mode, static_cast<float*>(dO));
    if (cudaDeviceSynchronize() != cudaSuccess || cudaMemcpy(out.data(), dO, out_n * 4, cudaMemcpyDeviceToHost) != cudaSuccess) {
      set_error(std::string("selftest_wgmma_row_shift: ") + cudaGetErrorString(cudaGetLastError()));
      rc = -2;
    }
  }
  cudaFree(dA);
  cudaFree(dW);
  cudaFree(dO);
  if (rc) return rc;
  *ok_shifts = 0;
  for (int r = 0; r <= 8; r++) {
    bool ok = true;
    for (int ks = 0; ks < 2; ks++)
      for (int m = 0; m < 64; m++)
        for (int n = 0; n < 8; n++) {
          float ref = 0.f;
          for (int k = 0; k < 16; k++) ref += Af[(r + m) * 32 + 16 * ks + k] * Wf[n * 32 + 16 * ks + k];
          if (out[((r * 2 + ks) * 64 + m) * 8 + n] != ref) ok = false;
        }
    if (ok) *ok_shifts |= 1u << r;
  }
  return 0;
}

__global__ void __launch_bounds__(256) split_kernel(const float* __restrict__ x, long long rows_out, int C, int ld_in,
                                                    int ld_out, int pool, int item_rows, const float* __restrict__ sc,
                                                    const float* __restrict__ sh, __nv_bfloat16* __restrict__ hi,
                                                    __nv_bfloat16* __restrict__ lo, const int* __restrict__ skip_flag) {
  if (skip_flag && *skip_flag != 0) return;
  const int q_per_row = ld_out >> 2;
  const long long n4 = rows_out * q_per_row;
  for (long long i = (long long)blockIdx.x * blockDim.x + threadIdx.x; i < n4; i += (long long)gridDim.x * blockDim.x) {
    const long long row = i / q_per_row;
    const int c = (int)(i - row * q_per_row) << 2;
    float4 v = make_float4(0.f, 0.f, 0.f, 0.f);
    if (c < C) {
      if (pool) {
        const float* p = x + (row * 3) * ld_in + c;
        const float4 a = *reinterpret_cast<const float4*>(p), b = *reinterpret_cast<const float4*>(p + ld_in),
                     d = *reinterpret_cast<const float4*>(p + 2 * ld_in);
        v = make_float4(fmaxf(fmaxf(a.x, b.x), d.x), fmaxf(fmaxf(a.y, b.y), d.y), fmaxf(fmaxf(a.z, b.z), d.z),
                        fmaxf(fmaxf(a.w, b.w), d.w));
      } else {
        v = *reinterpret_cast<const float4*>(x + row * ld_in + c);
      }
      if (sc) {
        const long long item = row / item_rows;
        const float4 s = *reinterpret_cast<const float4*>(sc + item * ld_in + c);
        const float4 h = *reinterpret_cast<const float4*>(sh + item * ld_in + c);
        v.x = leaky(fmaf(v.x, s.x, h.x)); v.y = leaky(fmaf(v.y, s.y, h.y));
        v.z = leaky(fmaf(v.z, s.z, h.z)); v.w = leaky(fmaf(v.w, s.w, h.w));
      }
    }
    uint16_t h0, h1, h2, h3, l0, l1, l2, l3;
    split_h16(v.x, h0, l0);
    split_h16(v.y, h1, l1);
    split_h16(v.z, h2, l2);
    split_h16(v.w, h3, l3);
    reinterpret_cast<uint2*>(hi)[i] = make_uint2(pack_u16x2(h0, h1), pack_u16x2(h2, h3));
    reinterpret_cast<uint2*>(lo)[i] = make_uint2(pack_u16x2(l0, l1), pack_u16x2(l2, l3));
  }
}

int launch_split_ex(const float* x, long long rows_out, int C, int ld_in, int ld_out, int pool, int item_rows,
                    const float* sc, const float* sh, void* hi, void* lo, cudaStream_t st, const int* skip_flag) {
  ProfScope _ps("split16", st);
  if (C % 4 || ld_in % 4 || ld_out % 4) {
    set_error("split: channel counts must be multiples of 4");
    return -1;
  }
  const long long n4 = rows_out * (ld_out / 4);
  const long long want = (n4 + 255) / 256;
  const int cap = usable_sms() * 16;
  const int grid = (int)(want < cap ? want : cap);
  split_kernel<<<grid, 256, 0, st>>>(x, rows_out, C, ld_in, ld_out, pool, item_rows, sc, sh,
                                     reinterpret_cast<__nv_bfloat16*>(hi), reinterpret_cast<__nv_bfloat16*>(lo), skip_flag);
  DG_LAUNCHED();
  return 0;
}

uint16_t host_f32_to_h16(float f) {
  uint32_t u;
  memcpy(&u, &f, 4);
  const uint32_t sign = (u >> 16) & 0x8000u;
  const uint32_t au = u & 0x7FFFFFFFu;
  if (au > 0x7F800000u) return (uint16_t)(sign | 0x7FFFu);
  if (au >= 0x477FF000u) return (uint16_t)(sign | 0x7BFFu);
  if (au < 0x33000001u) return (uint16_t)sign;
  const int e = (int)(au >> 23) - 127;
  uint32_t mant = (au & 0x7FFFFFu) | 0x800000u;
  int shift = e >= -14 ? 13 : 13 + (-14 - e);
  uint32_t q = mant >> shift;
  const uint32_t rem = mant & ((1u << shift) - 1u), half = 1u << (shift - 1);
  if (rem > half || (rem == half && (q & 1u))) q++;
  const uint32_t bits = e >= -14 ? (uint32_t)((e + 14) << 10) + q : q;
  return (uint16_t)(sign | bits);
}
float host_h16_to_f32(uint16_t h) {
  const uint32_t sign = ((uint32_t)h & 0x8000u) << 16, e = (h >> 10) & 31u, m = h & 0x3FFu;
  if (e == 0) {
    const float v = (float)m * 5.9604644775390625e-08f;
    return sign ? -v : v;
  }
  const uint32_t u = e == 31 ? (sign | 0x7F800000u | (m << 13)) : (sign | ((e + 112u) << 23) | (m << 13));
  float f;
  memcpy(&f, &u, 4);
  return f;
}

void split_weights_host(const float* w, int N, int Npad, int K, uint16_t* hi, uint16_t* lo, float scale) {
  for (size_t i = 0; i < (size_t)Npad * K; i++) hi[i] = lo[i] = 0;
  for (int n = 0; n < N; n++)
    for (int k = 0; k < K; k++) {
      const float f = w[(size_t)n * K + k] * scale;
      const uint16_t h = host_f32_to_h16(f);
      hi[(size_t)n * K + k] = h;
      lo[(size_t)n * K + k] = host_f32_to_h16(f - host_h16_to_f32(h));
    }
}

float weight_plane_scale(const float* w, size_t n) {
  float mx = 0.f;
  for (size_t i = 0; i < n; i++) {
    const float v = fabsf(w[i]);
    if (v > mx && v < 3.0e38f) mx = v;
  }
  if (!(mx > 0.f)) return 1.f;
  int e = 0;
  frexpf(mx, &e);
  int k = 13 - e;
  k = k > 40 ? 40 : (k < -40 ? -40 : k);
  return ldexpf(1.f, k);
}

}
```

diart_b200/csrc/tc_ptx.cuh:

```cuda
#pragma once
#include <cuda.h>
#include <cuda_bf16.h>
#include <stdint.h>

#include "dg_common.cuh"

namespace dg {

__device__ __forceinline__ uint32_t smem_u32(const void* p) { return (uint32_t)__cvta_generic_to_shared(p); }

__device__ __forceinline__ void mbar_init(uint64_t* bar, uint32_t count) {
  asm volatile("mbarrier.init.shared::cta.b64 [%0], %1;" ::"r"(smem_u32(bar)), "r"(count));
}
__device__ __forceinline__ void mbar_expect_tx(uint64_t* bar, uint32_t bytes) {
  asm volatile("mbarrier.arrive.expect_tx.shared::cta.b64 _, [%0], %1;" ::"r"(smem_u32(bar)), "r"(bytes) : "memory");
}
__device__ __forceinline__ void mbar_arrive(uint64_t* bar) {
  asm volatile("mbarrier.arrive.shared::cta.b64 _, [%0];" ::"r"(smem_u32(bar)) : "memory");
}
__device__ __forceinline__ bool mbar_try_wait(uint64_t* bar, uint32_t parity) {
  uint32_t ok;
  asm volatile(
      "{\n.reg .pred p;\nmbarrier.try_wait.parity.shared::cta.b64 p, [%1], %2;\nselp.u32 %0, 1, 0, p;\n}"
      : "=r"(ok)
      : "r"(smem_u32(bar)), "r"(parity)
      : "memory");
  return ok != 0;
}
__device__ __forceinline__ bool mbar_test_wait(uint64_t* bar, uint32_t parity) {
  uint32_t ok;
  asm volatile(
      "{\n.reg .pred p;\nmbarrier.test_wait.parity.shared::cta.b64 p, [%1], %2;\nselp.u32 %0, 1, 0, p;\n}"
      : "=r"(ok)
      : "r"(smem_u32(bar)), "r"(parity)
      : "memory");
  return ok != 0;
}
__device__ __forceinline__ void mbar_wait(uint64_t* bar, uint32_t parity) {
  if (mbar_try_wait(bar, parity)) return;
  const long long t0 = clock64();
  while (!mbar_try_wait(bar, parity)) {
    if (clock64() - t0 > 4000000000LL) __trap();
  }
}
__device__ __forceinline__ void tma_load_2d(void* smem_dst, const CUtensorMap* tmap, int c0, int c1, uint64_t* bar) {
  asm volatile(
      "cp.async.bulk.tensor.2d.shared::cluster.global.tile.mbarrier::complete_tx::bytes [%0], [%1, {%2, %3}], [%4];"
      ::"r"(smem_u32(smem_dst)), "l"(reinterpret_cast<uint64_t>(tmap)), "r"(c0), "r"(c1), "r"(smem_u32(bar))
      : "memory");
}
__device__ __forceinline__ void tma_load_4d(void* smem_dst, const CUtensorMap* tmap, int c0, int c1, int c2, int c3,
                                            uint64_t* bar) {
  asm volatile(
      "cp.async.bulk.tensor.4d.shared::cluster.global.tile.mbarrier::complete_tx::bytes [%0], [%1, {%2, %3, %4, %5}], [%6];"
      ::"r"(smem_u32(smem_dst)), "l"(reinterpret_cast<uint64_t>(tmap)), "r"(c0), "r"(c1), "r"(c2), "r"(c3), "r"(smem_u32(bar))
      : "memory");
}

__device__ __forceinline__ uint16_t f32_to_h16(float x) {
  uint16_t r;
  asm("cvt.rn.satfinite.f16.f32 %0, %1;" : "=h"(r) : "f"(x));
  return r;
}
__device__ __forceinline__ float h16_to_f32(uint16_t h) {
  float f;
  asm("cvt.f32.f16 %0, %1;" : "=f"(f) : "h"(h));
  return f;
}
__device__ __forceinline__ void split_h16(float x, uint16_t& hi, uint16_t& lo) {
  hi = f32_to_h16(x);
  lo = f32_to_h16(x - h16_to_f32(hi));
}
__device__ __forceinline__ uint32_t pack_u16x2(uint16_t a, uint16_t b) { return (uint32_t)a | ((uint32_t)b << 16); }

__device__ __forceinline__ void named_sync(int id, int n) { asm volatile("bar.sync %0, %1;" ::"r"(id), "r"(n) : "memory"); }
__device__ __forceinline__ void named_arrive(int id, int n) { asm volatile("bar.arrive %0, %1;" ::"r"(id), "r"(n) : "memory"); }
template <int R>
__device__ __forceinline__ void setmaxnreg_dec() { asm volatile("setmaxnreg.dec.sync.aligned.u32 %0;" ::"n"(R)); }
template <int R>
__device__ __forceinline__ void setmaxnreg_inc() { asm volatile("setmaxnreg.inc.sync.aligned.u32 %0;" ::"n"(R)); }

__device__ __forceinline__ void tma_store_2d(const CUtensorMap* tmap, const void* smem_src, int c0, int c1) {
  asm volatile("cp.async.bulk.tensor.2d.global.shared::cta.bulk_group [%0, {%2, %3}], [%1];"
               ::"l"(reinterpret_cast<uint64_t>(tmap)), "r"(smem_u32(smem_src)), "r"(c0), "r"(c1)
               : "memory");
}
__device__ __forceinline__ void fence_proxy_async_smem() { asm volatile("fence.proxy.async.shared::cta;" ::: "memory"); }
__device__ __forceinline__ void bulk_commit() { asm volatile("cp.async.bulk.commit_group;" ::: "memory"); }
__device__ __forceinline__ void bulk_wait_read_all() { asm volatile("cp.async.bulk.wait_group.read 0;" ::: "memory"); }
__device__ __forceinline__ void bulk_wait_all() { asm volatile("cp.async.bulk.wait_group 0;" ::: "memory"); }

__device__ __forceinline__ void st_shared_u32(uint32_t addr, uint32_t a) {
  asm volatile("st.shared.b32 [%0], %1;" ::"r"(addr), "r"(a) : "memory");
}
__device__ __forceinline__ void st_shared_v2(uint32_t addr, float a, float b) {
  asm volatile("st.shared.v2.f32 [%0], {%1, %2};" ::"r"(addr), "f"(a), "f"(b) : "memory");
}
__device__ __forceinline__ void st_shared_v4(uint32_t addr, uint32_t a, uint32_t b, uint32_t c, uint32_t d) {
  asm volatile("st.shared.v4.b32 [%0], {%1, %2, %3, %4};" ::"r"(addr), "r"(a), "r"(b), "r"(c), "r"(d) : "memory");
}


__device__ __forceinline__ uint64_t wg_desc(uint32_t smem_addr) {
  uint64_t d = 0;
  d |= (uint64_t)((smem_addr >> 4) & 0x3FFF);
  d |= (uint64_t)1 << 16;
  d |= (uint64_t)(1024 >> 4) << 32;
  d |= (uint64_t)1 << 62;
  return d;
}
__device__ __forceinline__ uint64_t wg_desc_sw64(uint32_t smem_addr) {
  uint64_t d = 0;
  d |= (uint64_t)((smem_addr >> 4) & 0x3FFF);
  d |= (uint64_t)1 << 16;
  d |= (uint64_t)(512 >> 4) << 32;
  d |= (uint64_t)2 << 62;
  return d;
}
__device__ __forceinline__ uint64_t wg_desc_plain(uint32_t smem_addr, uint32_t lbo, uint32_t sbo) {
  uint64_t d = 0;
  d |= (uint64_t)((smem_addr >> 4) & 0x3FFF);
  d |= (uint64_t)((lbo >> 4) & 0x3FFF) << 16;
  d |= (uint64_t)((sbo >> 4) & 0x3FFF) << 32;
  return d;
}
__device__ __forceinline__ void wg_fence() { asm volatile("wgmma.fence.sync.aligned;" ::: "memory"); }
__device__ __forceinline__ void wg_commit() { asm volatile("wgmma.commit_group.sync.aligned;" ::: "memory"); }
template <int N>
__device__ __forceinline__ void wg_wait() { asm volatile("wgmma.wait_group.sync.aligned %0;" ::"n"(N) : "memory"); }
template <int R>
__device__ __forceinline__ void wg_fence_acc(float (&d)[R]) {
#pragma unroll
  for (int i = 0; i < R; i++) asm volatile("" : "+f"(d[i])::"memory");
}

template <int N>
__device__ __forceinline__ void wgmma_ss(float (&d)[N / 2], uint64_t a, uint64_t b, uint32_t acc);
template <int N>
__device__ __forceinline__ void wgmma_rs(float (&d)[N / 2], const uint32_t (&a)[4], uint64_t b, uint32_t acc);

template <>
__device__ __forceinline__ void wgmma_ss<8>(float (&d)[4], uint64_t a, uint64_t b, uint32_t acc) {
  asm volatile("{\n.reg .pred p;\nsetp.ne.b32 p, %6, 0;\n"
               "wgmma.mma_async.sync.aligned.m64n8k16.f32.f16.f16 {%0, %1, %2, %3}, %4, %5, p, 1, 1, 0, 0;\n}"
               : "+f"(d[0]), "+f"(d[1]), "+f"(d[2]), "+f"(d[3])
               : "l"(a), "l"(b), "r"(acc));
}
template <>
__device__ __forceinline__ void wgmma_ss<16>(float (&d)[8], uint64_t a, uint64_t b, uint32_t acc) {
  asm volatile("{\n.reg .pred p;\nsetp.ne.b32 p, %10, 0;\n"
               "wgmma.mma_async.sync.aligned.m64n16k16.f32.f16.f16 {%0, %1, %2, %3, %4, %5, %6, %7}, %8, %9, p, 1, 1, 0, 0;\n}"
               : "+f"(d[0]), "+f"(d[1]), "+f"(d[2]), "+f"(d[3]), "+f"(d[4]), "+f"(d[5]), "+f"(d[6]), "+f"(d[7])
               : "l"(a), "l"(b), "r"(acc));
}
template <>
__device__ __forceinline__ void wgmma_ss<32>(float (&d)[16], uint64_t a, uint64_t b, uint32_t acc) {
  asm volatile("{\n.reg .pred p;\nsetp.ne.b32 p, %18, 0;\n"
               "wgmma.mma_async.sync.aligned.m64n32k16.f32.f16.f16 {%0, %1, %2, %3, %4, %5, %6, %7, %8, %9, %10, %11, %12, %13, %14, %15}, %16, %17, p, 1, 1, 0, 0;\n}"
               : "+f"(d[0]), "+f"(d[1]), "+f"(d[2]), "+f"(d[3]), "+f"(d[4]), "+f"(d[5]), "+f"(d[6]), "+f"(d[7]), "+f"(d[8]), "+f"(d[9]), "+f"(d[10]), "+f"(d[11]), "+f"(d[12]), "+f"(d[13]), "+f"(d[14]), "+f"(d[15])
               : "l"(a), "l"(b), "r"(acc));
}
template <>
__device__ __forceinline__ void wgmma_ss<64>(float (&d)[32], uint64_t a, uint64_t b, uint32_t acc) {
  asm volatile("{\n.reg .pred p;\nsetp.ne.b32 p, %34, 0;\n"
               "wgmma.mma_async.sync.aligned.m64n64k16.f32.f16.f16 {%0, %1, %2, %3, %4, %5, %6, %7, %8, %9, %10, %11, %12, %13, %14, %15, %16, %17, %18, %19, %20, %21, %22, %23, %24, %25, %26, %27, %28, %29, %30, %31}, %32, %33, p, 1, 1, 0, 0;\n}"
               : "+f"(d[0]), "+f"(d[1]), "+f"(d[2]), "+f"(d[3]), "+f"(d[4]), "+f"(d[5]), "+f"(d[6]), "+f"(d[7]), "+f"(d[8]), "+f"(d[9]), "+f"(d[10]), "+f"(d[11]), "+f"(d[12]), "+f"(d[13]), "+f"(d[14]), "+f"(d[15]), "+f"(d[16]), "+f"(d[17]), "+f"(d[18]), "+f"(d[19]), "+f"(d[20]), "+f"(d[21]), "+f"(d[22]), "+f"(d[23]), "+f"(d[24]), "+f"(d[25]), "+f"(d[26]), "+f"(d[27]), "+f"(d[28]), "+f"(d[29]), "+f"(d[30]), "+f"(d[31])
               : "l"(a), "l"(b), "r"(acc));
}
template <>
__device__ __forceinline__ void wgmma_ss<80>(float (&d)[40], uint64_t a, uint64_t b, uint32_t acc) {
  asm volatile("{\n.reg .pred p;\nsetp.ne.b32 p, %42, 0;\n"
               "wgmma.mma_async.sync.aligned.m64n80k16.f32.f16.f16 {%0, %1, %2, %3, %4, %5, %6, %7, %8, %9, %10, %11, %12, %13, %14, %15, %16, %17, %18, %19, %20, %21, %22, %23, %24, %25, %26, %27, %28, %29, %30, %31, %32, %33, %34, %35, %36, %37, %38, %39}, %40, %41, p, 1, 1, 0, 0;\n}"
               : "+f"(d[0]), "+f"(d[1]), "+f"(d[2]), "+f"(d[3]), "+f"(d[4]), "+f"(d[5]), "+f"(d[6]), "+f"(d[7]), "+f"(d[8]), "+f"(d[9]), "+f"(d[10]), "+f"(d[11]), "+f"(d[12]), "+f"(d[13]), "+f"(d[14]), "+f"(d[15]), "+f"(d[16]), "+f"(d[17]), "+f"(d[18]), "+f"(d[19]), "+f"(d[20]), "+f"(d[21]), "+f"(d[22]), "+f"(d[23]), "+f"(d[24]), "+f"(d[25]), "+f"(d[26]), "+f"(d[27]), "+f"(d[28]), "+f"(d[29]), "+f"(d[30]), "+f"(d[31]), "+f"(d[32]), "+f"(d[33]), "+f"(d[34]), "+f"(d[35]), "+f"(d[36]), "+f"(d[37]), "+f"(d[38]), "+f"(d[39])
               : "l"(a), "l"(b), "r"(acc));
}
template <>
__device__ __forceinline__ void wgmma_ss<128>(float (&d)[64], uint64_t a, uint64_t b, uint32_t acc) {
  asm volatile("{\n.reg .pred p;\nsetp.ne.b32 p, %66, 0;\n"
               "wgmma.mma_async.sync.aligned.m64n128k16.f32.f16.f16 {%0, %1, %2, %3, %4, %5, %6, %7, %8, %9, %10, %11, %12, %13, %14, %15, %16, %17, %18, %19, %20, %21, %22, %23, %24, %25, %26, %27, %28, %29, %30, %31, %32, %33, %34, %35, %36, %37, %38, %39, %40, %41, %42, %43, %44, %45, %46, %47, %48, %49, %50, %51, %52, %53, %54, %55, %56, %57, %58, %59, %60, %61, %62, %63}, %64, %65, p, 1, 1, 0, 0;\n}"
               : "+f"(d[0]), "+f"(d[1]), "+f"(d[2]), "+f"(d[3]), "+f"(d[4]), "+f"(d[5]), "+f"(d[6]), "+f"(d[7]), "+f"(d[8]), "+f"(d[9]), "+f"(d[10]), "+f"(d[11]), "+f"(d[12]), "+f"(d[13]), "+f"(d[14]), "+f"(d[15]), "+f"(d[16]), "+f"(d[17]), "+f"(d[18]), "+f"(d[19]), "+f"(d[20]), "+f"(d[21]), "+f"(d[22]), "+f"(d[23]), "+f"(d[24]), "+f"(d[25]), "+f"(d[26]), "+f"(d[27]), "+f"(d[28]), "+f"(d[29]), "+f"(d[30]), "+f"(d[31]), "+f"(d[32]), "+f"(d[33]), "+f"(d[34]), "+f"(d[35]), "+f"(d[36]), "+f"(d[37]), "+f"(d[38]), "+f"(d[39]), "+f"(d[40]), "+f"(d[41]), "+f"(d[42]), "+f"(d[43]), "+f"(d[44]), "+f"(d[45]), "+f"(d[46]), "+f"(d[47]), "+f"(d[48]), "+f"(d[49]), "+f"(d[50]), "+f"(d[51]), "+f"(d[52]), "+f"(d[53]), "+f"(d[54]), "+f"(d[55]), "+f"(d[56]), "+f"(d[57]), "+f"(d[58]), "+f"(d[59]), "+f"(d[60]), "+f"(d[61]), "+f"(d[62]), "+f"(d[63])
               : "l"(a), "l"(b), "r"(acc));
}
template <>
__device__ __forceinline__ void wgmma_rs<8>(float (&d)[4], const uint32_t (&a)[4], uint64_t b, uint32_t acc) {
  asm volatile("{\n.reg .pred p;\nsetp.ne.b32 p, %9, 0;\n"
               "wgmma.mma_async.sync.aligned.m64n8k16.f32.f16.f16 {%0, %1, %2, %3}, {%4, %5, %6, %7}, %8, p, 1, 1, 0;\n}"
               : "+f"(d[0]), "+f"(d[1]), "+f"(d[2]), "+f"(d[3])
               : "r"(a[0]), "r"(a[1]), "r"(a[2]), "r"(a[3]), "l"(b), "r"(acc));
}
template <>
__device__ __forceinline__ void wgmma_rs<16>(float (&d)[8], const uint32_t (&a)[4], uint64_t b, uint32_t acc) {
  asm volatile("{\n.reg .pred p;\nsetp.ne.b32 p, %13, 0;\n"
               "wgmma.mma_async.sync.aligned.m64n16k16.f32.f16.f16 {%0, %1, %2, %3, %4, %5, %6, %7}, {%8, %9, %10, %11}, %12, p, 1, 1, 0;\n}"
               : "+f"(d[0]), "+f"(d[1]), "+f"(d[2]), "+f"(d[3]), "+f"(d[4]), "+f"(d[5]), "+f"(d[6]), "+f"(d[7])
               : "r"(a[0]), "r"(a[1]), "r"(a[2]), "r"(a[3]), "l"(b), "r"(acc));
}

typedef CUresult (*EncodeTiledFn)(CUtensorMap*, CUtensorMapDataType, cuuint32_t, void*, const cuuint64_t*,
                                  const cuuint64_t*, const cuuint32_t*, const cuuint32_t*, CUtensorMapInterleave,
                                  CUtensorMapSwizzle, CUtensorMapL2promotion, CUtensorMapFloatOOBfill);

static inline EncodeTiledFn encode_fn() {
  static EncodeTiledFn fn = nullptr;
  if (!fn) {
    void* p = nullptr;
    cudaDriverEntryPointQueryResult q;
    if (cudaGetDriverEntryPoint("cuTensorMapEncodeTiled", &p, cudaEnableDefault, &q) == cudaSuccess &&
        q == cudaDriverEntryPointSuccess)
      fn = reinterpret_cast<EncodeTiledFn>(p);
  }
  return fn;
}

}
```

include/diart_b200.h:

```cpp
#ifndef DIART_B200_H
#define DIART_B200_H

#include <stddef.h>
#include <stdint.h>

#ifdef __cplusplus
extern "C" {
#endif

#define DG_OK 0
#define DG_EINVAL (-1)
#define DG_ECUDA (-2)
#define DG_EWEIGHT (-3)
#define DG_ENCCL (-4)

typedef struct dg_tensor {
  const char* name;
  const float* data;
  int64_t numel;
} dg_tensor;

typedef struct dg_seg dg_seg;
typedef struct dg_emb dg_emb;
typedef struct dg_cluster dg_cluster;
typedef struct dg_pipeline dg_pipeline;
typedef struct dg_post dg_post;
typedef struct dg_stream dg_stream;
typedef struct dg_sweep dg_sweep;
typedef struct dg_vad_sweep dg_vad_sweep;

const char* dg_last_error(void);
int dg_version(void);

int dg_seg_create(const dg_tensor* tensors, int n_tensors, int device, dg_seg** out);
int dg_seg_dims(const dg_seg* h, int num_samples, int* frames, int* speakers);
int dg_seg_set_powerset(dg_seg* h, int num_speakers, int max_per_frame);
int dg_seg_forward(dg_seg* h, const float* wav_dev , int B, int S,
                   float* seg_dev , void* stream);
int dg_seg_destroy(dg_seg* h);

int dg_emb_create(const dg_tensor* tensors, int n_tensors, int pool_mode, int device, dg_emb** out);
int dg_emb_dims(const dg_emb* h, int num_samples, int* frames, int* dimension);
int dg_emb_forward(dg_emb* h, const float* wav_dev , const float* weights_dev, int B, int S,
                   int F, int K, int normalize, float norm, float* out_dev, void* stream);
int dg_emb_forward_rows(dg_emb* h, const float* wav_dev , const float* weights_dev ,
                        int N, int S, int F, float* out_dev , void* stream);
int dg_emb_destroy(dg_emb* h);
int dg_emb_debug_trunk(dg_emb* h, const float* wav_dev, int U, int S, int stop_after, float* out_host, int64_t cap, int* dims);
int dg_seg_debug_stage(dg_seg* h, const float* wav_dev, int B, int S, int hop, int stage, float* out_host, int64_t cap, int* dims);
int dg_emb_debug_stage(dg_emb* h, const float* wav_dev, const float* weights_dev, int B, int S, int F, int K, int hop, int stage,
                       float* out_host, int64_t cap, int* dims);

int dg_osp(const float* seg_dev , int B, int F, int K, float gamma, float beta,
           int normalize, float* out_dev, void* stream);
int dg_normalize_embeddings(const float* emb_dev , int rows, int D, float norm,
                            float* out_dev, void* stream);

int dg_cluster_create(int max_speakers, int dim, double tau_active, double rho_update,
                      double delta_new, int device, dg_cluster** out);
int dg_cluster_set_metric(dg_cluster* h, int metric);
int dg_cluster_step(dg_cluster* h, const float* seg_dev , const float* emb_dev ,
                    int B, int F, int K, int32_t* map_dev, float* permuted_dev, void* stream);
int dg_cluster_reset(dg_cluster* h);
int dg_cluster_get_state(dg_cluster* h, double* centers_host, int32_t* active_host, int* initialized);
int dg_cluster_set_state(dg_cluster* h, const double* centers_host, const int32_t* active_host, int initialized);
int dg_cluster_destroy(dg_cluster* h);

int dg_pipeline_create(dg_seg* seg, dg_emb* emb, dg_cluster* clu, float gamma, float beta,
                       int normalize_weights, dg_pipeline** out);
int dg_pipeline_step(dg_pipeline* h, const float* wav_dev , int B, int S,
                     float* seg_dev , float* emb_dev ,
                     int32_t* map_dev , float* permuted_dev , void* stream);
int dg_pipeline_set_hop(dg_pipeline* h, int hop_samples);
int dg_pipeline_step_host(dg_pipeline* h, const float* wav_host, int B, int S, float* seg_host,
                          float* emb_host, int32_t* map_host, float* permuted_host );
int dg_pipeline_submit(dg_pipeline* h, const float* wav_dev , int B, int S,
                       void* stream);
int dg_pipeline_collect(dg_pipeline* h, const float** seg_dev, const float** emb_dev, const int32_t** map_dev,
                        void* stream);
int dg_pipeline_collect_copy(dg_pipeline* h, float* seg_dev, float* emb_dev, int32_t* map_dev, void* stream);
int dg_pipeline_submit_host(dg_pipeline* h, const float* wav_host , int B, int S);
int dg_pipeline_collect_host(dg_pipeline* h, float* seg_host, float* emb_host, int32_t* map_host);
int dg_pipeline_nets_sets(dg_pipeline* h, const float* wav_dev, int B, int S, int num_sets, const float* osp_host,
                          const int32_t* normalize_host, float* seg_dev, float* emb_dev, int64_t emb_set_stride, void* stream);
int dg_pipeline_destroy(dg_pipeline* h);

int dg_post_create(int frames, int local_speakers, int max_speakers, int num_windows, const double* hamming_host,
                   double tau, int device, dg_post** out);
int dg_post_step(dg_post* h, const float* seg_dev , const int32_t* map_dev , int B,
                 const int32_t* plan_host, int32_t* header_host, uint32_t* turns_host, int turn_cap_host, int* n_turns,
                 void* stream);
int dg_post_reset(dg_post* h);
int dg_post_destroy(dg_post* h);
int dg_pipeline_call_host(dg_pipeline* h, dg_post* post, const float* const* rows_host, int B, int S,
                          const int32_t* plan_host, int32_t* header_host, uint32_t* turns_host, int turn_cap_host,
                          int* n_turns, float* seg_host , int32_t* map_host );
int64_t dg_pipeline_last_call_h2d_bytes(const dg_pipeline* h);

int dg_sweep_create(int max_speakers, int dim, int frames, int local_speakers, int num_windows, const double* hamming_host,
                    int device, dg_sweep** out);
int dg_sweep_run(dg_sweep* h, const float* seg_dev, const float* emb_dev, int N, const double* params_host, int T,
                 const int32_t* plan_host, int32_t* maps_dev, double* centers_dev, int32_t* header_host, uint32_t* turns_host,
                 int turn_cap_host, int* n_turns, void* stream);
int dg_sweep_destroy(dg_sweep* h);
int dg_sweep_set_scored_regions(dg_sweep* h, int num_files, const double* rows_host, const int32_t* offsets_host);
int dg_vad_sweep_set_scored_regions(dg_vad_sweep* h, int num_files, const double* rows_host, const int32_t* offsets_host);
int dg_sweep_set_trial_sets(dg_sweep* h, int num_sets, const int32_t* trial_set_host, int T);
int dg_sweep_set_seeds(dg_sweep* h, int num_files, const int32_t* offsets_host, const double* centers_host);
int dg_sweep_set_identities(dg_sweep* h, int num_files, const int32_t* hyp_of_ref_host);
int dg_sweep_score(dg_sweep* h, const float* seg_dev, const float* emb_dev, int N, const double* params_host, int T,
                   const int32_t* plan_host, const double* out_start_host, const double* out_res_host, double shift,
                   double collar, const double* ref_host, const int32_t* ref_label_host, int S, int R,
                   double* components_host, int32_t* hyp_offsets_dev, double* hyp_segments_dev, int hyp_cap, void* stream);
int dg_sweep_run_files(dg_sweep* h, const float* seg_dev, const float* emb_dev, int N, int num_files,
                       const int32_t* chunk_offsets_host, const double* params_host, int T, const int32_t* plan_host,
                       int32_t* maps_dev, double* centers_dev, int32_t* header_host, uint32_t* turns_host, int turn_cap_host,
                       int* n_turns, void* stream);
int dg_sweep_score_files(dg_sweep* h, const float* seg_dev, const float* emb_dev, int N, int num_files,
                         const int32_t* chunk_offsets_host, const double* params_host, int T, const int32_t* plan_host,
                         const double* out_start_host, const double* out_res_host, const double* shifts_host, double collar,
                         const double* ref_host, const int32_t* ref_label_host, const int32_t* ref_offsets_host,
                         const int32_t* ref_label_counts_host, double* components_host, int32_t* hyp_offsets_dev,
                         double* hyp_segments_dev, int hyp_cap, void* stream);
int dg_sweep_state_order(int num_files, const int32_t* chunk_offsets_host, int T, int32_t* states_host);
int dg_sweep_run_latencies(dg_sweep* h, const float* seg_dev, const float* emb_dev, int N, int num_units,
                           const int32_t* unit_offsets_host, int num_virtual, int num_virtual_files, const int32_t* vchunk_host,
                           const int32_t* virtual_offsets_host, const double* params_host, int T, const int32_t* plan_host,
                           int32_t* maps_dev, int32_t* header_host, uint32_t* turns_host, int turn_cap_host, int* n_turns,
                           void* stream);
int dg_sweep_score_latencies(dg_sweep* h, const float* seg_dev, const float* emb_dev, int N, int num_units,
                             const int32_t* unit_offsets_host, int num_virtual, int num_virtual_files,
                             const int32_t* vchunk_host, const int32_t* virtual_offsets_host, const double* params_host, int T,
                             const int32_t* plan_host, const double* out_start_host, const double* out_res_host,
                             const double* shifts_host, double collar, const double* ref_host, const int32_t* ref_label_host,
                             const int32_t* ref_offsets_host, const int32_t* ref_label_counts_host, double* components_host,
                             void* stream);
int dg_sweep_check_latencies(int N, int num_units, const int32_t* unit_offsets_host, int num_virtual, int num_virtual_files,
                             const int32_t* vchunk_host, const int32_t* virtual_offsets_host, const int32_t* plan_host,
                             int num_windows, int frames);
int dg_vad_sweep_create(int frames, int local_speakers, int num_windows, const double* hamming_host, int device,
                        dg_vad_sweep** out);
int dg_vad_sweep_curve(dg_vad_sweep* h, const float* seg_dev, int N, int num_files, const int32_t* chunk_offsets_host,
                       const int32_t* plan_host, void* stream);
int dg_vad_sweep_curve_latencies(dg_vad_sweep* h, const float* seg_dev, int N, int num_units, const int32_t* unit_offsets_host,
                                 int num_virtual, int num_virtual_files, const int32_t* vchunk_host,
                                 const int32_t* virtual_offsets_host, const int32_t* plan_host, void* stream);
int dg_vad_sweep_run_files(dg_vad_sweep* h, const double* taus_host, int T, int32_t* header_host, uint32_t* turns_host,
                           int turn_cap_host, int* n_turns, void* stream);
int dg_vad_sweep_score_files(dg_vad_sweep* h, const double* taus_host, int T, const double* out_start_host,
                             const double* out_res_host, const double* shifts_host, double collar, const double* ref_host,
                             const int32_t* ref_offsets_host, double* components_host, void* stream);
int dg_vad_sweep_destroy(dg_vad_sweep* h);

int dg_stream_create(int chunk_samples, int step_samples, int max_windows, int device, dg_stream** out);
int dg_stream_push_host(dg_stream* h, const float* samples_host, int n);
int dg_stream_available(const dg_stream* h);
int dg_stream_windows(dg_stream* h, int B, float* wav_dev, void* stream);
int dg_stream_reset(dg_stream* h);
int dg_stream_destroy(dg_stream* h);
int dg_pipeline_submit_stream(dg_pipeline* h, dg_stream* stream, int B);
int dg_pipeline_call_stream(dg_pipeline* h, dg_post* post, dg_stream* stream, int B, const int32_t* plan_host,
                            int32_t* header_host, uint32_t* turns_host, int turn_cap_host, int* n_turns,
                            float* seg_host , int32_t* map_host );

typedef struct dg_multi dg_multi;
int dg_multi_create(dg_seg* seg, dg_emb* emb, int chunk_samples, int step_samples, int max_streams, int max_windows_per_stream,
                    int max_speakers, double tau, double rho, double delta, float gamma, float beta, int normalize_weights,
                    int num_windows, const double* hamming_host, dg_multi** out);
int dg_multi_open(dg_multi* h, int slot);
int dg_multi_close(dg_multi* h, int slot);
int dg_multi_push_host(dg_multi* h, int slot, const float* samples_host, int n);
int dg_multi_available(const dg_multi* h, int slot);
int dg_multi_step(dg_multi* h, const int32_t* plan_host, int n_rows, int32_t* counts_host, int32_t* header_host,
                  uint32_t* turns_host, int turn_cap_host, int* n_turns, float* seg_dev ,
                  float* emb_dev , int32_t* map_dev );
int dg_multi_last_step_ms(const dg_multi* h, float* ms);
int dg_multi_destroy(dg_multi* h);
typedef struct dg_resample dg_resample;
int dg_multi_add_rate(dg_multi* h, dg_resample* rs, int chunk_samples, int step_samples, int* rate_id);
int dg_multi_open_rate(dg_multi* h, int slot, int rate_id);
int dg_multi_open_config(dg_multi* h, int slot, int rate_id, int num_windows, const double params[3] );
int dg_multi_open_seeded(dg_multi* h, int slot, int rate_id, int num_windows, const double params[3] ,
                         const double* centers_host , int n);
int dg_multi_get_state(dg_multi* h, int slot, double* centers_host , int32_t* active_host ,
                       int* initialized);
typedef struct dg_gallery dg_gallery;
int dg_gallery_create(const double* centroids_host, int G, int D, int device, dg_gallery** out);
int dg_gallery_destroy(dg_gallery* g);
int dg_gallery_query(dg_gallery* g, const double* queries_dev , int Q, const int32_t* group_dev ,
                     const int32_t* claimed_dev , double threshold, int32_t* entry_dev ,
                     double* dist_dev , void* stream);
int dg_multi_set_gallery(dg_multi* h, dg_gallery* g, double threshold);
int dg_multi_set_slot_gallery(dg_multi* h, int slot, dg_gallery* g, double threshold);
int dg_multi_set_names(dg_multi* h, int slot, uint32_t named, const int32_t* claimed_host );
int dg_multi_last_names(const dg_multi* h, int32_t* out_host , int cap, int* n);
int dg_multi_last_windows(const dg_multi* h, float* wav_dev, int n_rows);
int dg_multi_export_bytes(const dg_multi* h, const int32_t* slots, int n, int64_t* bytes_out);
int dg_multi_export(dg_multi* h, const int32_t* slots, int n, int close, void* out_host, int64_t out_bytes);
int dg_multi_import(dg_multi* h, const void* blob_host, int64_t blob_bytes, int n, dg_gallery* const* gals,
                    int32_t* slots_out);
int dg_selftest_multi_transfer_host(const int32_t* geom, int n_ops, const int32_t* ops, const float* samples_host,
                                    int32_t* result, int src_slot, int patch, float* ring_out, float* yring_out, float* hist_out,
                                    int64_t cap, int64_t* info, char* message, int msg_cap);
int dg_selftest_multi_frames_host(int slots, int max_wps, int out_chunk, int out_step, int n_rates, const int32_t* rates,
                                  int n_ops, const int32_t* ops, int32_t* result, int64_t* records, int cap, int* n_records);
int dg_selftest_multi_staging_host(int slots, int C, int n_ops, const int32_t* ops, const float* samples_host, int32_t* result,
                                   float* rings_host);
int dg_selftest_gallery_plan_host(int n, const int32_t* slots, int n_keys, const int32_t* G, const double* thr,
                                  int32_t* groups_out, int32_t* segs_out, int32_t* work_out, int cap, int32_t* counts);
int dg_selftest_multi_gallery_host(int slots, int D, int M, int n_gal, const int32_t* gal, int n_ops, const double* ops,
                                   int32_t* result, char* messages, int msg_cap);
int dg_multi_create_vad(dg_seg* seg, int chunk_samples, int step_samples, int max_streams, int max_windows_per_stream,
                        double tau, int num_windows, const double* hamming_host, dg_multi** out);

typedef struct dg_resample dg_resample;
int dg_resample_create(int orig_rate, int new_rate, const float* taps_host, int width, int device, dg_resample** out);
int64_t dg_resample_out_len(const dg_resample* h, int64_t num_samples);
int dg_resample_forward(dg_resample* h, const float* in_dev, int B, int64_t L, float* out_dev, void* stream);
int dg_resample_destroy(dg_resample* h);
int dg_stream_create_resampled(int chunk_samples, int step_samples, dg_resample* rs, int max_windows, int device,
                               dg_stream** out);
int dg_stream_crop_host(dg_stream* h, int n, const int64_t* ranges_host, float* out_host);

int64_t dg_launch_count(void);
int dg_profile_enable(int enable);
int dg_selftest_gemm_tc(int M, int Cin, int KW, int dil, int N, int epi, float* max_abs_diff, float* out_rms);
int dg_selftest_gemm_tc_grid(int M, int Cin, int KW, int dil, int N, int epi, int* equal);
int dg_selftest_gemm_tc_bounds(int M, int Cin, int N, int epi, int* outside_unchanged, int* equal, int* refused);
int dg_selftest_wgmma_row_shift(int base_offset_mode, unsigned* ok_shifts);
int dg_selftest_gemm_tc_halo(int M, int Cin, int KW, int dil, int N, int epi, int* equal, int* halo);
int dg_selftest_split_f16_host(const float* x, long long n, unsigned short* hi, unsigned short* lo);
int dg_selftest_sinc_filters_host(const float* low_hz, const float* band_hz, float* filters);
int dg_selftest_fbank_tables_host(float* frame_operator, float* mel_banks);
int dg_profile_report(char* buf, int cap);

int dg_cluster_record_len(const dg_cluster* h);
int dg_cluster_export_delta(dg_cluster* h, double* record_dev, void* stream);
int dg_cluster_merge(dg_cluster* h, const double* records_dev , int world, int rank,
                     int32_t* maps_dev , int n_maps, void* stream);
int dg_pipeline_identity_export(dg_pipeline* h, double* record_dev, void* stream);
int dg_pipeline_identity_merge(dg_pipeline* h, const double* records_dev, int world, int rank, void* stream);

#ifdef __cplusplus
}
#endif
#endif
```

Before: 22720.

## Add warp-specialized ping-pong maxpool3 conv GEMM with TMA producer and 112-row tiles

Adds a warp-specialized tensor-core kernel for the maxpool3 conv epilogue. One producer warpgroup issues TMA loads of weights and halo tiles and hands out tiles through a dynamic atomic tile counter. Two consumer warpgroups alternate in ping-pong order with named barriers, so one group's MMA overlaps the other group's pooling epilogue. Tiles are transposed to 112 output rows using m64n112 wgmma, with weights as the A operand. The shared pooling epilogue is factored into a helper, and selftests for B-row shift and pool3 correctness are added. The extra register, barrier and scheduling complexity risks hurting throughput if the ws path's conditions do not suit the real shapes.

```diff
diff --git a/diart_b200/_lib.py b/diart_b200/_lib.py
--- a/diart_b200/_lib.py
+++ b/diart_b200/_lib.py
@@ -30,6 +30,9 @@
     "dg_selftest_gemm_tc_bounds": (C.c_int, [C.c_int, C.c_int, C.c_int, C.c_int, C.POINTER(C.c_int), C.POINTER(C.c_int),
                                              C.POINTER(C.c_int)]),
     "dg_selftest_wgmma_row_shift": (C.c_int, [C.c_int, C.POINTER(C.c_uint)]),
+    "dg_selftest_wgmma_b_row_shift": (C.c_int, [C.c_int, C.POINTER(C.c_uint)]),
+    "dg_selftest_gemm_tc_pool3_simt": (C.c_int, [C.c_int, C.c_int, C.c_int, C.c_int, C.c_int, C.POINTER(C.c_float),
+                                                 C.POINTER(C.c_float), C.POINTER(C.c_int)]),
     "dg_selftest_gemm_tc_halo": (C.c_int, [C.c_int, C.c_int, C.c_int, C.c_int, C.c_int, C.c_int, C.POINTER(C.c_int),
                                            C.POINTER(C.c_int)]),
     "dg_selftest_split_f16_host": (C.c_int, [_P, C.c_longlong, _P, _P]),
diff --git a/diart_b200/csrc/api.cu b/diart_b200/csrc/api.cu
--- a/diart_b200/csrc/api.cu
+++ b/diart_b200/csrc/api.cu
@@ -308,6 +308,71 @@
     return DG_EINVAL;
   }
   return selftest_wgmma_row_shift(base_offset_mode, ok_shifts) ? DG_ECUDA : DG_OK;
+}
+
+extern "C" int dg_selftest_wgmma_b_row_shift(int base_offset_mode, unsigned* ok_shifts) {
+  if (base_offset_mode < 0 || base_offset_mode > 1 || !ok_shifts) {
+    set_error("dg_selftest_wgmma_b_row_shift: bad arguments");
+    return DG_EINVAL;
+  }
+  return selftest_wgmma_b_row_shift(base_offset_mode, ok_shifts) ? DG_ECUDA : DG_OK;
+}
+
+extern "C" int dg_selftest_gemm_tc_pool3_simt(int M, int Cin, int KW, int dil, int N, float* max_abs_diff, float* out_rms,
+                                              int* ws) {
+  if (M < 888 || M % 888 || Cin < 16 || Cin % 16 || Cin > 128 || KW < 2 || KW > 9 || dil < 1 || N < 1 || N > 64 || N % 4 ||
+      !max_abs_diff || !out_rms || !ws) {
+    set_error("dg_selftest_gemm_tc_pool3_simt: bad arguments");
+    return DG_EINVAL;
+  }
+  const int K = KW * Cin, item_rows = 888, tile_rows = gemm_tc_pool3_tile_rows(item_rows);
+  const long long m_tiles = (M + tile_rows - 1) / tile_rows, tail = (long long)(KW - 1) * dil;
+  uint32_t seed = 4242u;
+  auto rnd = [&]() {
+    seed = seed * 1664525u + 1013904223u;
+    return ((seed >> 8) & 0xFFFF) / 65536.f - 0.5f;
+  };
+  std::vector<float> A((size_t)(M + tail) * Cin, 0.f), Wkn((size_t)K * N), Wnk((size_t)N * K), bias(N);
+  for (size_t i = 0; i < (size_t)M * Cin; i++) A[i] = 2.f * rnd();
+  for (int k = 0; k < K; k++)
+    for (int n = 0; n < N; n++) Wkn[(size_t)k * N + n] = Wnk[(size_t)n * K + k] = 0.25f * rnd();
+  for (auto& v : bias) v = rnd();
+  DevBuf dA, dWkn, dB, dAh, dAl, dC0, dP, dPart;
+  WeightPlanes dW;
+  if (upload(dA, A) || upload(dWkn, Wkn) || upload(dB, bias) || upload_split(dW, Wnk, N, 64, K)) return DG_ECUDA;
+  if (dAh.ensure((size_t)M * Cin * 2) || dAl.ensure((size_t)M * Cin * 2) || dC0.ensure((size_t)M * N * 4) ||
+      dP.ensure((size_t)(M / 3) * N * 4) || dPart.ensure((size_t)m_tiles * 2 * TC_POOL3_SLOTS * N * 4))
+    return DG_ECUDA;
+  int rc;
+  GemmArgs g{};
+  g.A = dA.as<float>(); g.lda = Cin; g.Cin = Cin; g.KW = KW; g.dil = dil; g.Mtot = M + tail; g.M = M;
+  g.W = dWkn.as<float>(); g.ldw = N; g.N = N; g.bias = dB.as<float>(); g.C = dC0.as<float>(); g.ldc = N; g.epi = EPI_BIAS;
+  g.tag = "selftest_simt";
+  if ((rc = launch_gemm(g, nullptr))) return rc;
+  if ((rc = launch_split_ex(dA.as<float>(), M, Cin, Cin, Cin, 0, 1, nullptr, nullptr, dAh.p, dAl.p, nullptr))) return rc;
+  TcGemm t{};
+  t.A_hi = dAh.p; t.A_lo = dAl.p; t.lda = Cin; t.Cin = Cin; t.KW = KW; t.dil = dil; t.Mtot = M; t.M = M;
+  t.N = N; t.bias = dB.as<float>(); t.out_f32 = dP.as<float>(); t.ldc = N; t.epi = 5; t.tag = "selftest_tc_pool3";
+  t.pool_part = dPart.as<float>(); t.pool_item_rows = item_rows; t.pool3_T = item_rows / 3 - 2; t.pool3_tile_rows = tile_rows;
+  if ((rc = set_weights(t, dW))) return rc;
+  *ws = gemm_tc_ws(t) ? 1 : 0;
+  if ((rc = launch_gemm_tc(t, nullptr))) return rc;
+  DG_CUDA(cudaDeviceSynchronize());
+  std::vector<float> c0((size_t)M * N), p1((size_t)(M / 3) * N);
+  DG_CUDA(cudaMemcpy(c0.data(), dC0.p, c0.size() * 4, cudaMemcpyDeviceToHost));
+  DG_CUDA(cudaMemcpy(p1.data(), dP.p, p1.size() * 4, cudaMemcpyDeviceToHost));
+  double md = 0, ss = 0;
+  for (long long r = 0; r < M / 3; r++)
+    for (int n = 0; n < N; n++) {
+      const float* x = &c0[(size_t)(3 * r) * N + n];
+      const double ref = std::max(std::max(x[0], x[N]), x[2 * N]);
+      const double d = fabs(ref - (double)p1[(size_t)r * N + n]);
+      if (!(d <= md)) md = d;
+      ss += ref * ref;
+    }
+  *max_abs_diff = (float)md;
+  *out_rms = (float)sqrt(ss / p1.size());
+  return DG_OK;
 }
 
 extern "C" int dg_selftest_gemm_tc_halo(int M, int Cin, int KW, int dil, int N, int epi, int* equal, int* halo) {
diff --git a/diart_b200/csrc/dg_common.cuh b/diart_b200/csrc/dg_common.cuh
--- a/diart_b200/csrc/dg_common.cuh
+++ b/diart_b200/csrc/dg_common.cuh
@@ -148,7 +148,9 @@
 }
 int launch_gemm_tc(const TcGemm& g, cudaStream_t st);
 bool gemm_tc_halo(const TcGemm& g);
+bool gemm_tc_ws(const TcGemm& g);
 int selftest_wgmma_row_shift(int base_offset_mode, unsigned* ok_shifts);
+int selftest_wgmma_b_row_shift(int base_offset_mode, unsigned* ok_shifts);
 int launch_split_ex(const float* x, long long rows_out, int C, int ld_in, int ld_out, int pool, int item_rows,
                     const float* sc, const float* sh, void* hi, void* lo, cudaStream_t st, const int* skip_flag = nullptr);
 void split_weights_host(const float* w, int N, int Npad, int K, uint16_t* hi, uint16_t* lo, float scale = 1.f);
diff --git a/diart_b200/csrc/gemm_tc.cu b/diart_b200/csrc/gemm_tc.cu
--- a/diart_b200/csrc/gemm_tc.cu
+++ b/diart_b200/csrc/gemm_tc.cu
@@ -221,6 +221,58 @@
     }
 }
 
+template <bool STG_IN_DSM = false>
+__device__ __forceinline__ void tc_maxpool3_cols(const TcArgs& a, const float* dsm, float* stg, const float* bias_c,
+                                                 long long mt, int nc, int et, int bar) {
+  {
+    const int col = et & 31, rg = et >> 5, n = nc + col;
+    const long long first = mt * (long long)a.tile_rows;
+    const long long item0 = first / a.pool_item_rows;
+    const long long nxt = (item0 + 1) * a.pool_item_rows;
+    const int brow3 = nxt - first < a.tile_rows ? (int)(nxt - first) / 3 : a.tile_rows / 3;
+    const long long p_first = first / 3;
+    const int f0 = (int)(p_first - item0 * (a.pool_item_rows / 3));
+    const long long Mp = a.M / 3;
+    const float bias = bias_c[col];
+    auto pooled = [&](int pr) {
+      return fmaxf(fmaxf(dsm[(3 * pr) * 33 + col], dsm[(3 * pr + 1) * 33 + col]), dsm[(3 * pr + 2) * 33 + col]);
+    };
+    const float piv0 = pooled(0), piv1 = pooled(brow3 < a.tile_rows / 3 ? brow3 : 0);
+    float s1[2] = {0.f, 0.f}, s2[2] = {0.f, 0.f};
+    for (int pr = rg; pr < a.tile_rows / 3; pr += 4) {
+      const float v = pooled(pr);
+      const int sg = pr >= brow3 ? 1 : 0;
+      const int frame = sg ? pr - brow3 : f0 + pr;
+      const long long P = p_first + pr;
+      if (P < Mp) {
+        if (n < a.N) a.out_f32[P * a.ldc + n] = v + bias;
+        if (frame < a.pool3_T) {
+          const float dv = v - (sg ? piv1 : piv0);
+          s1[sg] += dv;
+          s2[sg] = fmaf(dv, dv, s2[sg]);
+        }
+      }
+    }
+    if (STG_IN_DSM) named_sync(bar, 128);
+#pragma unroll
+    for (int sg = 0; sg < 2; sg++) {
+      stg[((rg * 2 + sg) * 2 + 0) * 32 + col] = s1[sg];
+      stg[((rg * 2 + sg) * 2 + 1) * 32 + col] = s2[sg];
+    }
+    if (rg == 0 && n < a.N)
+#pragma unroll
+      for (int sg = 0; sg < 2; sg++) a.pool_part[(((size_t)mt * 2 + sg) * TC_POOL3_SLOTS + 2) * a.N + n] = sg ? piv1 : piv0;
+  }
+  named_sync(bar, 128);
+  {
+    const int col = et & 31, q = et >> 5, sg = q >> 1, j = q & 1, n = nc + col;
+    const float tot = ((stg[((0 * 2 + sg) * 2 + j) * 32 + col] + stg[((1 * 2 + sg) * 2 + j) * 32 + col]) +
+                       stg[((2 * 2 + sg) * 2 + j) * 32 + col]) + stg[((3 * 2 + sg) * 2 + j) * 32 + col];
+    if (n < a.N) a.pool_part[(((size_t)mt * 2 + sg) * TC_POOL3_SLOTS + j) * a.N + n] = tot;
+  }
+  named_sync(bar, 128);
+}
+
 template <int BN, int EPI>
 __device__ __forceinline__ void tc_pool_epilogue_tile(const TcArgs& a, float* params, float* chunk, float* pool_stage,
                                                  const float (&acc)[2][BN / 2], int bar, long long mt, int n0, int quad,
@@ -349,54 +401,7 @@
           continue;
         }
         if (EPI == TC_MAXPOOL3) {
-          const float* dsm = chunk + (c - c0) / 32 * (128 * 33);
-          float* stg = pool_stage;
-          {
-            const int col = et & 31, rg = et >> 5, n = n0 + c + col;
-            const long long first = mt * (long long)a.tile_rows;
-            const long long item0 = first / a.pool_item_rows;
-            const long long nxt = (item0 + 1) * a.pool_item_rows;
-            const int brow3 = nxt - first < a.tile_rows ? (int)(nxt - first) / 3 : a.tile_rows / 3;
-            const long long p_first = first / 3;
-            const int f0 = (int)(p_first - item0 * (a.pool_item_rows / 3));
-            const long long Mp = a.M / 3;
-            const float bias = params[c + col];
-            auto pooled = [&](int pr) {
-              return fmaxf(fmaxf(dsm[(3 * pr) * 33 + col], dsm[(3 * pr + 1) * 33 + col]), dsm[(3 * pr + 2) * 33 + col]);
-            };
-            const float piv0 = pooled(0), piv1 = pooled(brow3 < a.tile_rows / 3 ? brow3 : 0);
-            float s1[2] = {0.f, 0.f}, s2[2] = {0.f, 0.f};
-            for (int pr = rg; pr < a.tile_rows / 3; pr += 4) {
-              const float v = pooled(pr);
-              const int sg = pr >= brow3 ? 1 : 0;
-              const int frame = sg ? pr - brow3 : f0 + pr;
-              const long long P = p_first + pr;
-              if (P < Mp) {
-                if (n < a.N) a.out_f32[P * a.ldc + n] = v + bias;
-                if (frame < a.pool3_T) {
-                  const float dv = v - (sg ? piv1 : piv0);
-                  s1[sg] += dv;
-                  s2[sg] = fmaf(dv, dv, s2[sg]);
-                }
-              }
-            }
-#pragma unroll
-            for (int sg = 0; sg < 2; sg++) {
-              stg[((rg * 2 + sg) * 2 + 0) * 32 + col] = s1[sg];
-              stg[((rg * 2 + sg) * 2 + 1) * 32 + col] = s2[sg];
-            }
-            if (rg == 0 && n < a.N)
-#pragma unroll
-              for (int sg = 0; sg < 2; sg++) a.pool_part[(((size_t)mt * 2 + sg) * TC_POOL3_SLOTS + 2) * a.N + n] = sg ? piv1 : piv0;
-          }
-          named_sync(bar, 128);
-          {
-            const int col = et & 31, q = et >> 5, sg = q >> 1, j = q & 1, n = n0 + c + col;
-            const float tot = ((stg[((0 * 2 + sg) * 2 + j) * 32 + col] + stg[((1 * 2 + sg) * 2 + j) * 32 + col]) +
-                               stg[((2 * 2 + sg) * 2 + j) * 32 + col]) + stg[((3 * 2 + sg) * 2 + j) * 32 + col];
-            if (n < a.N) a.pool_part[(((size_t)mt * 2 + sg) * TC_POOL3_SLOTS + j) * a.N + n] = tot;
-          }
-          named_sync(bar, 128);
+          tc_maxpool3_cols(a, chunk + (c - c0) / 32 * (128 * 33), pool_stage, params + c, mt, n0 + c, et, bar);
           continue;
         }
       }
@@ -666,6 +671,155 @@
   if (tc_box_store(EPI) && et == 0) bulk_wait_all();
 }
 
+constexpr int TCW_N = 112;
+struct TcWsSmem {
+  static constexpr int W_BOX = 64 * TC_BK * 2;
+  static constexpr int BAR_BYTES = 128;
+  static constexpr int CHUNK_FLOATS = TCW_N * 33;
+  static constexpr int STAGE_FLOATS = 64 + 2 * CHUNK_FLOATS;
+  __host__ static int halo_rows(int KW, int dil) { return (TCW_N + (KW - 1) * dil + 7) / 8 * 8; }
+  __host__ static int w_plane_bytes(int K) { return (K + TC_BK - 1) / TC_BK * W_BOX; }
+  __host__ static int op_bytes(int cin, int KW, int dil) {
+    return 2 * w_plane_bytes(KW * cin) + 2 * TcSmem<64>::halo_bytes(cin, halo_rows(KW, dil));
+  }
+  __host__ static int total(int op) { return op + BAR_BYTES + STAGE_FLOATS * 4 + 1024; }
+};
+
+__global__ void __launch_bounds__(TC_THREADS, 1)
+gemm_tc_ws_kernel(const __grid_constant__ CUtensorMap tmA_hi, const __grid_constant__ CUtensorMap tmA_lo,
+                  const __grid_constant__ CUtensorMap tmW_hi, const __grid_constant__ CUtensorMap tmW_lo, TcArgs a) {
+  using S = TcWsSmem;
+  extern __shared__ unsigned char smem_raw[];
+  unsigned char* smem = reinterpret_cast<unsigned char*>((reinterpret_cast<uintptr_t>(smem_raw) + 1023) & ~uintptr_t(1023));
+  const int w_plane = a.wblocks * S::W_BOX;
+  unsigned char* halo = smem + 2 * w_plane;
+  uint64_t* bars = reinterpret_cast<uint64_t*>(smem + a.op_bytes);
+  uint64_t* w_full = bars;
+  uint64_t* tile_full = bars + 1;
+  uint64_t* tile_empty = bars + 3;
+  uint64_t* halo_full = bars + 5;
+  uint64_t* halo_empty = bars + 7;
+  volatile int* tile_idx = reinterpret_cast<volatile int*>(bars + 9);
+  float* bias_s = reinterpret_cast<float*>(reinterpret_cast<unsigned char*>(bars) + S::BAR_BYTES);
+
+  const int warp = __shfl_sync(0xffffffffu, (int)(threadIdx.x >> 5), 0), lane = threadIdx.x & 31;
+  const int wg = warp >> 2;
+  const int num_tiles = a.m_tiles;
+  const int halo_box = a.halo_rows * 64, halo_cb = (a.cin + 31) / 32;
+
+  if (threadIdx.x == 0) {
+    mbar_init(w_full, 1);
+    for (int c = 0; c < 2; c++) {
+      mbar_init(&tile_full[c], 1);
+      mbar_init(&tile_empty[c], 128);
+      mbar_init(&halo_full[c], 1);
+      mbar_init(&halo_empty[c], 1);
+    }
+    asm volatile("fence.mbarrier_init.release.cluster;" ::: "memory");
+  }
+  if (threadIdx.x < 64) bias_s[threadIdx.x] = (int)threadIdx.x < a.N && a.bias ? a.bias[threadIdx.x] : 0.f;
+  __syncthreads();
+
+  if (wg == 0) {
+    setmaxnreg_dec<40>();
+    if (threadIdx.x == 0) {
+      mbar_expect_tx(w_full, 2 * w_plane);
+      for (int b = 0; b < a.wblocks; b++) {
+        tma_load_2d(smem + b * S::W_BOX, &tmW_hi, b * TC_BK, 0, w_full);
+        tma_load_2d(smem + w_plane + b * S::W_BOX, &tmW_lo, b * TC_BK, 0, w_full);
+      }
+      for (int i = 0, tile = blockIdx.x;; i++) {
+        const int c = i & 1;
+        if (tile < num_tiles) {
+          mbar_wait(&halo_empty[c], ((i >> 1) & 1) ^ 1);
+          unsigned char* hs = halo + c * a.halo_bytes;
+          const int r0 = tile * a.tile_rows;
+          mbar_expect_tx(&halo_full[c], 2 * halo_cb * halo_box);
+          for (int cb = 0; cb < halo_cb; cb++) {
+            tma_load_2d(hs + cb * halo_box, &tmA_hi, cb * TC_BK, r0, &halo_full[c]);
+            tma_load_2d(hs + (halo_cb + cb) * halo_box, &tmA_lo, cb * TC_BK, r0, &halo_full[c]);
+          }
+        }
+        mbar_wait(&tile_empty[c], ((i >> 1) & 1) ^ 1);
+        if (tile >= num_tiles) {
+          tile_idx[c] = -1;
+          mbar_arrive(&tile_full[c]);
+          mbar_wait(&tile_empty[c ^ 1], (((i + 1) >> 1) & 1) ^ 1);
+          tile_idx[c ^ 1] = -2;
+          mbar_arrive(&tile_full[c ^ 1]);
+          break;
+        }
+        tile_idx[c] = tile;
+        mbar_arrive(&tile_full[c]);
+        tile = (int)gridDim.x + (int)atomicAdd(&a.tile_ctr[0], 1u);
+      }
+      __threadfence();
+      if (atomicAdd(&a.tile_ctr[1], 1u) == gridDim.x - 1) {
+        atomicExch(&a.tile_ctr[0], 0u);
+        atomicExch(&a.tile_ctr[1], 0u);
+      }
+    }
+    return;
+  }
+  setmaxnreg_inc<232>();
+  const int c = wg - 1, quad = warp & 3, et = threadIdx.x - 128 * wg;
+  const int bar = 1 + c, turn = 3 + c, turn_other = 3 + (c ^ 1);
+  float* chunk = bias_s + 64 + c * S::CHUNK_FLOATS;
+  if (c == 1) named_arrive(3, 256);
+  const int ksteps = a.KW * a.cin / 16;
+  const uint32_t w_s = smem_u32(smem), hs = smem_u32(halo + c * a.halo_bytes);
+  mbar_wait(w_full, 0);
+  for (int n = 0;; n++) {
+    mbar_wait(&tile_full[c], n & 1);
+    const int tile = tile_idx[c];
+    mbar_arrive(&tile_empty[c]);
+    named_sync(turn, 256);
+    if (tile < 0) {
+      if (tile == -1) named_arrive(turn_other, 256);
+      break;
+    }
+    float acc[TCW_N / 2];
+#pragma unroll
+    for (int i = 0; i < TCW_N / 2; i++) acc[i] = 0.f;
+    mbar_wait(&halo_full[c], n & 1);
+    uint32_t htap = 0;
+    int hch = 0;
+    wg_fence_acc(acc);
+    wg_fence();
+    for (int s = 0; s < ksteps; s++) {
+      const uint32_t wa = w_s + (uint32_t)(s >> 1) * S::W_BOX + (uint32_t)(s & 1) * 32;
+      const uint64_t w_hi = wg_desc_sw64(wa), w_lo = wg_desc_sw64(wa + w_plane);
+      const uint32_t xa = hs + (uint32_t)(hch >> 5) * halo_box + (uint32_t)(hch & 31) * 2 + htap;
+      const uint64_t x_hi = wg_desc_sw64(xa), x_lo = wg_desc_sw64(xa + halo_cb * halo_box);
+      hch += 16;
+      const bool next_tap = hch == a.cin;
+      hch = next_tap ? 0 : hch;
+      htap += next_tap ? a.dil * 64 : 0;
+      wgmma_ss<TCW_N>(acc, w_hi, x_lo, s != 0);
+      wgmma_ss<TCW_N>(acc, w_lo, x_hi, 1);
+      wgmma_ss<TCW_N>(acc, w_hi, x_hi, 1);
+    }
+    wg_commit();
+    named_arrive(turn_other, 256);
+    wg_wait<0>();
+    wg_fence_acc(acc);
+    if (et == 0) mbar_arrive(&halo_empty[c]);
+    const uint32_t frag = smem_u32(chunk) + 4 * (2 * (lane & 3) * 33 + 16 * (quad & 1) + (lane >> 2));
+#pragma unroll
+    for (int c0 = 0; c0 < 64; c0 += 32) {
+      if ((quad >> 1) == (c0 >> 5)) {
+#pragma unroll
+        for (int j = 0; j < TCW_N / 8; j++)
+#pragma unroll
+          for (int e = 0; e < 4; e++)
+            st_shared_u32(frag + 4 * ((8 * j + (e & 1)) * 33 + 8 * (e >> 1)), __float_as_uint(acc[4 * j + e] * a.acc_scale));
+      }
+      named_sync(bar, 128);
+      tc_maxpool3_cols<true>(a, chunk, chunk, bias_s + c0, tile, c0, et, bar);
+    }
+  }
+}
+
 static int make_map(CUtensorMap* m, const void* base, long long rows, int cols, int ld, int box_cols, int box_rows,
                     bool f32 = false) {
   EncodeTiledFn fn = encode_fn();
@@ -730,15 +884,22 @@
 template <int BN>
 static int tc_halo_smem(const TcGemm& g) { return TcSmem<BN>::total(g.epi, TcSmem<BN>::halo_op_bytes(g.Cin, tc_halo_rows(g))); }
 
+bool gemm_tc_ws(const TcGemm& g) {
+  if (g.epi != TC_MAXPOOL3 || g.tap_boxes || g.tap_off || g.KW < 2 || g.dil < 1 || g.Cin % 16 || g.Cin > 128 ||
+      g.pool3_tile_rows > TCW_N || TcWsSmem::halo_rows(g.KW, g.dil) > 256)
+    return false;
+  return TcWsSmem::total(TcWsSmem::op_bytes(g.Cin, g.KW, g.dil)) <= TC_SMEM_MAX;
+}
+
 bool gemm_tc_halo(const TcGemm& g) {
   if (g.tap_boxes || g.epi == TC_CONV2D || g.tap_off || g.KW < 2 || g.dil < 1 || g.Cin % 16 || g.Cin > 128 ||
       tc_halo_rows(g) > 256)
     return false;
-  return (tc_bn(g) == 64 ? tc_halo_smem<64>(g) : tc_halo_smem<128>(g)) <= TC_SMEM_MAX;
-}
-
-static int tc_setup(const TcGemm& g, int bn, int epi, bool halo, CUtensorMap* maps, TcArgs& a) {
-  const int Ktot = g.KW * g.Cin, bk = TC_BK, a_rows = halo ? tc_halo_rows(g) : TC_BM;
+  return gemm_tc_ws(g) || (tc_bn(g) == 64 ? tc_halo_smem<64>(g) : tc_halo_smem<128>(g)) <= TC_SMEM_MAX;
+}
+
+static int tc_setup(const TcGemm& g, int bn, int epi, bool halo, CUtensorMap* maps, TcArgs& a, bool ws = false) {
+  const int Ktot = g.KW * g.Cin, bk = TC_BK, a_rows = ws ? TcWsSmem::halo_rows(g.KW, g.dil) : (halo ? tc_halo_rows(g) : TC_BM);
   if (make_map(&maps[0], g.A_hi, g.Mtot, g.Cin, g.lda, bk, a_rows) || make_map(&maps[1], g.A_lo, g.Mtot, g.Cin, g.lda, bk, a_rows) ||
       make_map(&maps[2], g.W_hi, g.Npad, Ktot, Ktot, bk, bn) || make_map(&maps[3], g.W_lo, g.Npad, Ktot, Ktot, bk, bn))
     return -2;
@@ -765,7 +926,12 @@
   a.res_lo = reinterpret_cast<const __nv_bfloat16*>(g.res_lo);
   a.pool_w = g.pool_w; a.pool_part = g.pool_part; a.pool_item_rows = g.pool_item_rows; a.pool_K = g.pool_K; a.pool_T = g.pool_T;
   a.cin = g.Cin;
-  if (halo) {
+  if (ws) {
+    a.halo_rows = a_rows;
+    a.wblocks = (Ktot + bk - 1) / bk;
+    a.halo_bytes = TcSmem<64>::halo_bytes(g.Cin, a_rows);
+    a.op_bytes = TcWsSmem::op_bytes(g.Cin, g.KW, g.dil);
+  } else if (halo) {
     a.halo_rows = a_rows;
     a.wblocks = (Ktot + bk - 1) / bk;
     a.halo_bytes = bn == 64 ? TcSmem<64>::halo_bytes(g.Cin, a_rows) : TcSmem<128>::halo_bytes(g.Cin, a_rows);
@@ -799,6 +965,18 @@
   return 0;
 }
 
+static int launch_tc_ws(const TcGemm& g, cudaStream_t st) {
+  CUtensorMap m[6];
+  TcArgs a;
+  if (tc_setup(g, 64, TC_MAXPOOL3, true, m, a, true) || !(a.tile_ctr = tile_counter(st))) return -2;
+  static bool attr_done[64] = {};
+  if (first_use_on_device(attr_done))
+    DG_CUDA(cudaFuncSetAttribute(gemm_tc_ws_kernel, cudaFuncAttributeMaxDynamicSharedMemorySize, TC_SMEM_MAX));
+  gemm_tc_ws_kernel<<<tc_grid(a), TC_THREADS, TcWsSmem::total(a.op_bytes), st>>>(m[0], m[1], m[2], m[3], a);
+  DG_LAUNCHED();
+  return 0;
+}
+
 template <int BN, int EPI>
 static int launch_tc(const TcGemm& g, cudaStream_t st) {
   return gemm_tc_halo(g) ? launch_tc<BN, EPI, true>(g, st) : launch_tc<BN, EPI, false>(g, st);
@@ -848,6 +1026,7 @@
       set_error("gemm_tc (maxpool3): needs 64 output channels and tiles of 3..126 rows (a multiple of 3) that divide the item");
       return -1;
     }
+    if (gemm_tc_ws(g)) return launch_tc_ws(g, st);
     return launch_tc<64, TC_MAXPOOL3>(g, st);
   }
   if (g.Npad == 64 && g.epi == TC_BIAS_F32) return launch_tc<64, TC_BIAS_F32>(g, st);
@@ -937,6 +1116,89 @@
           float ref = 0.f;
           for (int k = 0; k < 16; k++) ref += Af[(r + m) * 32 + 16 * ks + k] * Wf[n * 32 + 16 * ks + k];
           if (out[((r * 2 + ks) * 64 + m) * 8 + n] != ref) ok = false;
+        }
+    if (ok) *ok_shifts |= 1u << r;
+  }
+  return 0;
+}
+
+__global__ void __launch_bounds__(128) wgmma_b_row_shift_kernel(const __grid_constant__ CUtensorMap tmA,
+                                                                const __grid_constant__ CUtensorMap tmB, int base_offset_mode,
+                                                                float* out) {
+  __shared__ __align__(1024) unsigned char sm[64 * 64 + 72 * 64];
+  __shared__ uint64_t bar;
+  if (threadIdx.x == 0) {
+    mbar_init(&bar, 1);
+    asm volatile("fence.mbarrier_init.release.cluster;" ::: "memory");
+  }
+  __syncthreads();
+  if (threadIdx.x == 0) {
+    mbar_expect_tx(&bar, sizeof(sm));
+    tma_load_2d(sm, &tmA, 0, 0, &bar);
+    tma_load_2d(sm + 64 * 64, &tmB, 0, 0, &bar);
+  }
+  mbar_wait(&bar, 0);
+  const int w = threadIdx.x >> 5, l = threadIdx.x & 31;
+  for (int r = 0; r <= 8; r++) {
+    for (int ks = 0; ks < 2; ks++) {
+      const uint32_t sb = smem_u32(sm + 64 * 64) + r * 64 + ks * 32;
+      uint64_t db = wg_desc_sw64(sb);
+      if (base_offset_mode) db |= (uint64_t)((sb >> 7) & 7) << 49;
+      const uint64_t da = wg_desc_sw64(smem_u32(sm) + ks * 32);
+      float d[32];
+      for (int i = 0; i < 32; i++) d[i] = 0.f;
+      wg_fence_acc(d);
+      wg_fence();
+      wgmma_ss<64>(d, da, db, 0);
+      wg_commit();
+      wg_wait<0>();
+      wg_fence_acc(d);
+      for (int i = 0; i < 32; i++)
+        out[((r * 2 + ks) * 64 + 16 * w + l / 4 + 8 * ((i / 2) % 2)) * 64 + 8 * (i / 4) + 2 * (l % 4) + i % 2] = d[i];
+    }
+  }
+}
+
+int selftest_wgmma_b_row_shift(int base_offset_mode, unsigned* ok_shifts) {
+  std::vector<uint16_t> A(64 * 32), B(72 * 32);
+  std::vector<float> Af(A.size()), Bf(B.size());
+  for (size_t i = 0; i < A.size(); i++) Af[i] = (float)((int)((i * 5 + i / 32) % 7) - 3);
+  for (size_t i = 0; i < B.size(); i++) Bf[i] = (float)((int)((i * 7 + i / 32 * 3) % 9) - 4);
+  for (size_t i = 0; i < A.size(); i++) A[i] = host_f32_to_h16(Af[i]);
+  for (size_t i = 0; i < B.size(); i++) B[i] = host_f32_to_h16(Bf[i]);
+  void *dA = nullptr, *dB = nullptr, *dO = nullptr;
+  const size_t out_n = 9 * 2 * 64 * 64;
+  int rc = 0;
+  CUtensorMap mA, mB;
+  if (cudaMalloc(&dA, A.size() * 2) != cudaSuccess || cudaMalloc(&dB, B.size() * 2) != cudaSuccess ||
+      cudaMalloc(&dO, out_n * 4) != cudaSuccess ||
+      cudaMemcpy(dA, A.data(), A.size() * 2, cudaMemcpyHostToDevice) != cudaSuccess ||
+      cudaMemcpy(dB, B.data(), B.size() * 2, cudaMemcpyHostToDevice) != cudaSuccess) {
+    set_error("selftest_wgmma_b_row_shift: device buffers");
+    rc = -2;
+  }
+  if (!rc && (make_map(&mA, dA, 64, 32, 32, 32, 64) || make_map(&mB, dB, 72, 32, 32, 32, 72))) rc = -2;
+  std::vector<float> out(out_n);
+  if (!rc) {
+    wgmma_b_row_shift_kernel<<<1, 128>>>(mA, mB, base_offset_mode, static_cast<float*>(dO));
+    if (cudaDeviceSynchronize() != cudaSuccess || cudaMemcpy(out.data(), dO, out_n * 4, cudaMemcpyDeviceToHost) != cudaSuccess) {
+      set_error(std::string("selftest_wgmma_b_row_shift: ") + cudaGetErrorString(cudaGetLastError()));
+      rc = -2;
+    }
+  }
+  cudaFree(dA);
+  cudaFree(dB);
+  cudaFree(dO);
+  if (rc) return rc;
+  *ok_shifts = 0;
+  for (int r = 0; r <= 8; r++) {
+    bool ok = true;
+    for (int ks = 0; ks < 2; ks++)
+      for (int m = 0; m < 64; m++)
+        for (int n = 0; n < 64; n++) {
+          float ref = 0.f;
+          for (int k = 0; k < 16; k++) ref += Af[m * 32 + 16 * ks + k] * Bf[(r + n) * 32 + 16 * ks + k];
+          if (out[((r * 2 + ks) * 64 + m) * 64 + n] != ref) ok = false;
         }
     if (ok) *ok_shifts |= 1u << r;
   }
diff --git a/diart_b200/csrc/tc_ptx.cuh b/diart_b200/csrc/tc_ptx.cuh
--- a/diart_b200/csrc/tc_ptx.cuh
+++ b/diart_b200/csrc/tc_ptx.cuh
@@ -172,6 +172,13 @@
   asm volatile("{\n.reg .pred p;\nsetp.ne.b32 p, %42, 0;\n"
                "wgmma.mma_async.sync.aligned.m64n80k16.f32.f16.f16 {%0, %1, %2, %3, %4, %5, %6, %7, %8, %9, %10, %11, %12, %13, %14, %15, %16, %17, %18, %19, %20, %21, %22, %23, %24, %25, %26, %27, %28, %29, %30, %31, %32, %33, %34, %35, %36, %37, %38, %39}, %40, %41, p, 1, 1, 0, 0;\n}"
                : "+f"(d[0]), "+f"(d[1]), "+f"(d[2]), "+f"(d[3]), "+f"(d[4]), "+f"(d[5]), "+f"(d[6]), "+f"(d[7]), "+f"(d[8]), "+f"(d[9]), "+f"(d[10]), "+f"(d[11]), "+f"(d[12]), "+f"(d[13]), "+f"(d[14]), "+f"(d[15]), "+f"(d[16]), "+f"(d[17]), "+f"(d[18]), "+f"(d[19]), "+f"(d[20]), "+f"(d[21]), "+f"(d[22]), "+f"(d[23]), "+f"(d[24]), "+f"(d[25]), "+f"(d[26]), "+f"(d[27]), "+f"(d[28]), "+f"(d[29]), "+f"(d[30]), "+f"(d[31]), "+f"(d[32]), "+f"(d[33]), "+f"(d[34]), "+f"(d[35]), "+f"(d[36]), "+f"(d[37]), "+f"(d[38]), "+f"(d[39])
+               : "l"(a), "l"(b), "r"(acc));
+}
+template <>
+__device__ __forceinline__ void wgmma_ss<112>(float (&d)[56], uint64_t a, uint64_t b, uint32_t acc) {
+  asm volatile("{\n.reg .pred p;\nsetp.ne.b32 p, %58, 0;\n"
+               "wgmma.mma_async.sync.aligned.m64n112k16.f32.f16.f16 {%0, %1, %2, %3, %4, %5, %6, %7, %8, %9, %10, %11, %12, %13, %14, %15, %16, %17, %18, %19, %20, %21, %22, %23, %24, %25, %26, %27, %28, %29, %30, %31, %32, %33, %34, %35, %36, %37, %38, %39, %40, %41, %42, %43, %44, %45, %46, %47, %48, %49, %50, %51, %52, %53, %54, %55}, %56, %57, p, 1, 1, 0, 0;\n}"
+               : "+f"(d[0]), "+f"(d[1]), "+f"(d[2]), "+f"(d[3]), "+f"(d[4]), "+f"(d[5]), "+f"(d[6]), "+f"(d[7]), "+f"(d[8]), "+f"(d[9]), "+f"(d[10]), "+f"(d[11]), "+f"(d[12]), "+f"(d[13]), "+f"(d[14]), "+f"(d[15]), "+f"(d[16]), "+f"(d[17]), "+f"(d[18]), "+f"(d[19]), "+f"(d[20]), "+f"(d[21]), "+f"(d[22]), "+f"(d[23]), "+f"(d[24]), "+f"(d[25]), "+f"(d[26]), "+f"(d[27]), "+f"(d[28]), "+f"(d[29]), "+f"(d[30]), "+f"(d[31]), "+f"(d[32]), "+f"(d[33]), "+f"(d[34]), "+f"(d[35]), "+f"(d[36]), "+f"(d[37]), "+f"(d[38]), "+f"(d[39]), "+f"(d[40]), "+f"(d[41]), "+f"(d[42]), "+f"(d[43]), "+f"(d[44]), "+f"(d[45]), "+f"(d[46]), "+f"(d[47]), "+f"(d[48]), "+f"(d[49]), "+f"(d[50]), "+f"(d[51]), "+f"(d[52]), "+f"(d[53]), "+f"(d[54]), "+f"(d[55])
                : "l"(a), "l"(b), "r"(acc));
 }
 template <>
diff --git a/include/diart_b200.h b/include/diart_b200.h
--- a/include/diart_b200.h
+++ b/include/diart_b200.h
@@ -228,7 +228,9 @@
 int dg_selftest_gemm_tc_grid(int M, int Cin, int KW, int dil, int N, int epi, int* equal);
 int dg_selftest_gemm_tc_bounds(int M, int Cin, int N, int epi, int* outside_unchanged, int* equal, int* refused);
 int dg_selftest_wgmma_row_shift(int base_offset_mode, unsigned* ok_shifts);
+int dg_selftest_wgmma_b_row_shift(int base_offset_mode, unsigned* ok_shifts);
 int dg_selftest_gemm_tc_halo(int M, int Cin, int KW, int dil, int N, int epi, int* equal, int* halo);
+int dg_selftest_gemm_tc_pool3_simt(int M, int Cin, int KW, int dil, int N, float* max_abs_diff, float* out_rms, int* ws);
 int dg_selftest_split_f16_host(const float* x, long long n, unsigned short* hi, unsigned short* lo);
 int dg_selftest_sinc_filters_host(const float* low_hz, const float* band_hz, float* filters);
 int dg_selftest_fbank_tables_host(float* frame_operator, float* mel_banks);
```

Result: faster. 23540, median of 6 (+3.6%).
